# 4ment/physher

Measured on AMD Instinct MI355X. Metric: lnL+gradient evals/sec, 1000-taxon GTR+G4 fp64, 1e6 site patterns, higher is better.
Workload: dtype f64

## Files before the change

### include/physher_amd.h

```cpp
#ifndef PHYSHER_AMD_H
#define PHYSHER_AMD_H

#include <stddef.h>
#include <stdint.h>

#ifdef __cplusplus
extern "C" {
#endif

typedef struct phyamd_engine phyamd_engine;

enum {
	PHYAMD_OK = 0,
	PHYAMD_EINVAL = -1,
	PHYAMD_EDEVICE = -2,
	PHYAMD_ENOMEM = -3,
	PHYAMD_EUNSUPPORTED = -4
};

enum { PHYAMD_RESCALE_NEVER = 0, PHYAMD_RESCALE_ALWAYS = 1, PHYAMD_RESCALE_AUTO = 2 };

enum {
	PHYAMD_GRAD_FOLD_ROOT_FREQS = 1,
	PHYAMD_GRAD_COMPAT_SCALED = 2
};

typedef struct {
	int32_t tip_count;
	int32_t pattern_count;
	int32_t state_count;
	int32_t category_count;
	int32_t device;
	int32_t rescale;
	int64_t max_device_bytes;
	void *stream;
} phyamd_config;

int phyamd_create(const phyamd_config *cfg, phyamd_engine **out);
int phyamd_create_sharded(const phyamd_config *cfg, int32_t device_count, const int32_t *device_ids, phyamd_engine **out);
int phyamd_shard_count(phyamd_engine *e);
void phyamd_destroy(phyamd_engine *e);
const char *phyamd_last_error(void);
int phyamd_abi_version(void);

int phyamd_set_tip_states(phyamd_engine *e, int tip, const uint8_t *states);
int phyamd_set_tip_partials(phyamd_engine *e, int tip, const double *partials);
int phyamd_set_pattern_weights(phyamd_engine *e, const double *weights );

int phyamd_compress_patterns(int device , int32_t taxon_count, int64_t site_count, const uint8_t *const *rows,
                             const uint8_t *symbol_codes , int32_t *pattern_count, uint8_t *patterns, double *weights);

int phyamd_set_topology(phyamd_engine *e, const int32_t *left, const int32_t *right , int root);
int phyamd_set_branch_lengths(phyamd_engine *e, const double *lengths );

int phyamd_set_branch_length(phyamd_engine *e, int node, double length);
int phyamd_update_all_nodes(phyamd_engine *e);

int phyamd_store(phyamd_engine *e);
int phyamd_restore(phyamd_engine *e);

int phyamd_set_eigen(phyamd_engine *e, const double *eval, const double *evec, const double *ivec);
int phyamd_set_frequencies(phyamd_engine *e, const double *freqs );
int phyamd_set_category_rates(phyamd_engine *e, const double *rates , const double *proportions );
int phyamd_set_node_matrices(phyamd_engine *e, int node, const double *matrices);
int phyamd_set_matrices(phyamd_engine *e, const double *matrices);
int phyamd_set_rate_matrix(phyamd_engine *e, const double *Q);

int phyamd_log_likelihood(phyamd_engine *e, double *lnl);
int phyamd_gradient(phyamd_engine *e, int flags, double *lnl, double *cat_gradient);
int phyamd_branch_gradient(phyamd_engine *e, int flags, const double *rates_without_mu , double *lnl,
                           double *branch_gradient);
int phyamd_log_likelihood_device(phyamd_engine *e, double *device_out);
int phyamd_gradient_device(phyamd_engine *e, int flags, double *device_out);
int phyamd_root_invariant_term(phyamd_engine *e, double *out);

#define PHYAMD_MAX_PARAMETERS 2048
int phyamd_set_rate_matrix_derivatives(phyamd_engine *e, int count, const double *dQ);
int phyamd_parameter_gradient(phyamd_engine *e, int flags, double *lnl, double *cat_gradient, double *parameter_gradient);
int phyamd_parameter_gradient_device(phyamd_engine *e, int flags, double *device_out);
int phyamd_root_frequency_term(phyamd_engine *e, double *out );
int phyamd_branch_log_likelihood(phyamd_engine *e, int node, double length, double *lnl, double *d1, double *d2);
int phyamd_branch_hessian_diagonal(phyamd_engine *e, int flags, double *lnl, double *d1, double *d2);
int phyamd_branch_hessian_diagonal_device(phyamd_engine *e, int flags, double *device_out);
int phyamd_gradient_batch(phyamd_engine *e, int flags, int32_t count, const double *branch_lengths, double *lnl, double *cat_gradient);
int phyamd_gradient_batch_trees(phyamd_engine *e, int flags, int32_t count, const int32_t *left, const int32_t *right,
                                const int32_t *roots, const double *branch_lengths, double *lnl, double *cat_gradient);
typedef struct { int32_t items_fast, items_sequential, chunks; int64_t scratch_bytes; double ms; } phyamd_batch_profile;
int phyamd_get_batch_profile(phyamd_engine *e, phyamd_batch_profile *out);
int phyamd_nni_log_likelihoods(phyamd_engine *e, int flags, const double *central_lengths ,
                               double *lnl , double *d1 , double *d2 );
typedef struct { int32_t candidates; int64_t scratch_bytes; double ms; } phyamd_nni_profile;
int phyamd_get_nni_profile(phyamd_engine *e, phyamd_nni_profile *out);
int phyamd_spr_log_likelihoods(phyamd_engine *e, int flags, int32_t count, const int32_t *prune ,
                               double *lnl );
typedef struct { int32_t prunes, chunks; int64_t candidates, scratch_bytes; double ms; } phyamd_spr_profile;
int phyamd_get_spr_profile(phyamd_engine *e, phyamd_spr_profile *out);
int phyamd_state_posteriors(phyamd_engine *e, int flags, int32_t count, const int32_t *nodes ,
                            double *posteriors , uint8_t *states );
int phyamd_site_rate_posteriors(phyamd_engine *e, double *posteriors , double *mean_rates );
int phyamd_branch_hessian(phyamd_engine *e, int flags, double *lnl, double *gradient , double *hessian );
typedef struct { int32_t chunks; int64_t pairs, scratch_bytes; double ms; } phyamd_hessian_profile;
int phyamd_get_hessian_profile(phyamd_engine *e, phyamd_hessian_profile *out);
int phyamd_synchronize(phyamd_engine *e);

int phyamd_get_pattern_log_likelihoods(phyamd_engine *e, double *out );
int phyamd_get_partials(phyamd_engine *e, int node, int upper, double *out);
int phyamd_get_node_matrices(phyamd_engine *e, int node, int derivative, double *out );
int phyamd_post_order_parks(int32_t tip_count, const int32_t *left , const int32_t *right, int32_t root, int32_t second_slot,
                            int32_t *out , int32_t capacity);
int phyamd_is_rescaling(phyamd_engine *e);
int phyamd_set_rescaling(phyamd_engine *e, int policy);
int phyamd_set_keep_partials(phyamd_engine *e, int on);

typedef struct {
	double matrices_ms, lower_ms, upper_ms, reduce_ms;
	int32_t lower_launches, upper_launches;
	int64_t device_bytes;
	int32_t tiles;
} phyamd_profile;
int phyamd_set_reduction_levels(phyamd_engine *e, int levels);
int phyamd_set_profiling(phyamd_engine *e, int on);
int phyamd_get_profile(phyamd_engine *e, phyamd_profile *out);

#ifdef __cplusplus
}
#endif
#endif
```

### physher_amd/_lib.py

```python
from __future__ import annotations

import ctypes as C
import os

_HERE = os.path.dirname(os.path.abspath(__file__))
LIB_PATH = os.environ.get("PHYAMD_LIB") or os.path.join(_HERE, "libphysher_amd.so")

ABI_VERSION = 5

OK, EINVAL, EDEVICE, ENOMEM, EUNSUPPORTED = 0, -1, -2, -3, -4
RESCALE_NEVER, RESCALE_ALWAYS, RESCALE_AUTO = 0, 1, 2
GRAD_FOLD_ROOT_FREQS, GRAD_COMPAT_SCALED = 1, 2


class Config(C.Structure):
    _fields_ = [
        ("tip_count", C.c_int32), ("pattern_count", C.c_int32), ("state_count", C.c_int32),
        ("category_count", C.c_int32), ("device", C.c_int32), ("rescale", C.c_int32),
        ("max_device_bytes", C.c_int64), ("stream", C.c_void_p),
    ]


class Profile(C.Structure):
    _fields_ = [
        ("matrices_ms", C.c_double), ("lower_ms", C.c_double), ("upper_ms", C.c_double), ("reduce_ms", C.c_double),
        ("lower_launches", C.c_int32), ("upper_launches", C.c_int32), ("device_bytes", C.c_int64), ("tiles", C.c_int32),
    ]


class NniProfile(C.Structure):
    _fields_ = [("candidates", C.c_int32), ("scratch_bytes", C.c_int64), ("ms", C.c_double)]


class SprProfile(C.Structure):
    _fields_ = [("prunes", C.c_int32), ("chunks", C.c_int32), ("candidates", C.c_int64), ("scratch_bytes", C.c_int64), ("ms", C.c_double)]


class HessianProfile(C.Structure):
    _fields_ = [("chunks", C.c_int32), ("pairs", C.c_int64), ("scratch_bytes", C.c_int64), ("ms", C.c_double)]


class BatchProfile(C.Structure):
    _fields_ = [
        ("items_fast", C.c_int32), ("items_sequential", C.c_int32), ("chunks", C.c_int32), ("scratch_bytes", C.c_int64), ("ms", C.c_double),
    ]


_P = C.c_void_p
SYMBOLS = [
    ("phyamd_create", C.c_int, [C.POINTER(Config), C.POINTER(_P)]),
    ("phyamd_create_sharded", C.c_int, [C.POINTER(Config), C.c_int32, _P, C.POINTER(_P)]),
    ("phyamd_shard_count", C.c_int, [_P]),
    ("phyamd_destroy", None, [_P]),
    ("phyamd_last_error", C.c_char_p, []),
    ("phyamd_abi_version", C.c_int, []),
    ("phyamd_set_tip_states", C.c_int, [_P, C.c_int, _P]),
    ("phyamd_set_tip_partials", C.c_int, [_P, C.c_int, _P]),
    ("phyamd_set_pattern_weights", C.c_int, [_P, _P]),
    ("phyamd_set_topology", C.c_int, [_P, _P, _P, C.c_int]),
    ("phyamd_set_branch_lengths", C.c_int, [_P, _P]),
    ("phyamd_set_branch_length", C.c_int, [_P, C.c_int, C.c_double]),
    ("phyamd_update_all_nodes", C.c_int, [_P]),
    ("phyamd_set_eigen", C.c_int, [_P, _P, _P, _P]),
    ("phyamd_set_frequencies", C.c_int, [_P, _P]),
    ("phyamd_set_category_rates", C.c_int, [_P, _P, _P]),
    ("phyamd_set_node_matrices", C.c_int, [_P, C.c_int, _P]),
    ("phyamd_set_matrices", C.c_int, [_P, _P]),
    ("phyamd_set_rate_matrix", C.c_int, [_P, _P]),
    ("phyamd_log_likelihood", C.c_int, [_P, C.POINTER(C.c_double)]),
    ("phyamd_gradient", C.c_int, [_P, C.c_int, C.POINTER(C.c_double), _P]),
    ("phyamd_branch_gradient", C.c_int, [_P, C.c_int, _P, C.POINTER(C.c_double), _P]),
    ("phyamd_gradient_device", C.c_int, [_P, C.c_int, _P]),
    ("phyamd_log_likelihood_device", C.c_int, [_P, _P]),
    ("phyamd_root_invariant_term", C.c_int, [_P, C.POINTER(C.c_double)]),
    ("phyamd_set_rate_matrix_derivatives", C.c_int, [_P, C.c_int, _P]),
    ("phyamd_parameter_gradient", C.c_int, [_P, C.c_int, C.POINTER(C.c_double), _P, _P]),
    ("phyamd_parameter_gradient_device", C.c_int, [_P, C.c_int, _P]),
    ("phyamd_root_frequency_term", C.c_int, [_P, _P]),
    ("phyamd_branch_log_likelihood", C.c_int, [_P, C.c_int, C.c_double, C.POINTER(C.c_double), C.POINTER(C.c_double), C.POINTER(C.c_double)]),
    ("phyamd_branch_hessian_diagonal", C.c_int, [_P, C.c_int, C.POINTER(C.c_double), _P, _P]),
    ("phyamd_branch_hessian_diagonal_device", C.c_int, [_P, C.c_int, _P]),
    ("phyamd_gradient_batch", C.c_int, [_P, C.c_int, C.c_int32, _P, _P, _P]),
    ("phyamd_gradient_batch_trees", C.c_int, [_P, C.c_int, C.c_int32, _P, _P, _P, _P, _P, _P]),
    ("phyamd_get_batch_profile", C.c_int, [_P, C.POINTER(BatchProfile)]),
    ("phyamd_nni_log_likelihoods", C.c_int, [_P, C.c_int, _P, _P, _P, _P]),
    ("phyamd_get_nni_profile", C.c_int, [_P, C.POINTER(NniProfile)]),
    ("phyamd_spr_log_likelihoods", C.c_int, [_P, C.c_int, C.c_int32, _P, _P]),
    ("phyamd_get_spr_profile", C.c_int, [_P, C.POINTER(SprProfile)]),
    ("phyamd_state_posteriors", C.c_int, [_P, C.c_int, C.c_int32, _P, _P, _P]),
    ("phyamd_site_rate_posteriors", C.c_int, [_P, _P, _P]),
    ("phyamd_branch_hessian", C.c_int, [_P, C.c_int, _P, _P, _P]),
    ("phyamd_get_hessian_profile", C.c_int, [_P, C.POINTER(HessianProfile)]),
    ("phyamd_synchronize", C.c_int, [_P]),
    ("phyamd_get_pattern_log_likelihoods", C.c_int, [_P, _P]),
    ("phyamd_get_partials", C.c_int, [_P, C.c_int, C.c_int, _P]),
    ("phyamd_get_node_matrices", C.c_int, [_P, C.c_int, C.c_int, _P]),
    ("phyamd_post_order_parks", C.c_int, [C.c_int32, _P, _P, C.c_int32, C.c_int32, _P, C.c_int32]),
    ("phyamd_is_rescaling", C.c_int, [_P]),
    ("phyamd_set_rescaling", C.c_int, [_P, C.c_int]),
    ("phyamd_set_keep_partials", C.c_int, [_P, C.c_int]),
    ("phyamd_set_reduction_levels", C.c_int, [_P, C.c_int]),
    ("phyamd_set_profiling", C.c_int, [_P, C.c_int]),
    ("phyamd_get_profile", C.c_int, [_P, C.POINTER(Profile)]),
    ("phyamd_store", C.c_int, [_P]),
    ("phyamd_restore", C.c_int, [_P]),
    ("phyamd_compress_patterns", C.c_int, [C.c_int, C.c_int32, C.c_int64, _P, _P, C.POINTER(C.c_int32), _P, _P]),
]

_lib = None


def load():
    global _lib
    if _lib is not None:
        return _lib
    if not os.path.exists(LIB_PATH):
        raise ImportError(f"{LIB_PATH} is missing: build the HIP engine first (make -C physher_amd/csrc); there is no CPU fallback")
    lib = C.CDLL(LIB_PATH)
    for name, res, args in SYMBOLS:
        fn = getattr(lib, name)
        fn.restype = res
        fn.argtypes = args
    if lib.phyamd_abi_version() != ABI_VERSION:
        raise ImportError(f"ABI mismatch: library {lib.phyamd_abi_version()} != binding {ABI_VERSION}")
    _lib = lib
    return lib


class EngineError(RuntimeError):
    def __init__(self, code, message):
        super().__init__(f"physher_amd engine error {code}: {message}")
        self.code = code
```

### physher_amd/csrc/phyamd_abi.inc

```

#include <condition_variable>
#include <functional>
#include <mutex>
#include <thread>

namespace {

class ShardWorkers {
public:
	explicit ShardWorkers(int n) : done_(0), generation_(0), stop_(false) {
		for (int i = 0; i < n; i++) threads_.emplace_back([this, i] { loop(i); });
	}
	~ShardWorkers() {
		{
			std::lock_guard<std::mutex> lk(m_);
			stop_ = true;
			generation_++;
		}
		cv_.notify_all();
		for (auto &t : threads_) t.join();
	}
	void run(const std::function<void(int)> &fn) {
		std::unique_lock<std::mutex> lk(m_);
		fn_ = &fn;
// ... 542 lines not shown
int phyamd_state_posteriors(phyamd_engine *g, int flags, int32_t count, const int32_t *nodes, double *posteriors, uint8_t *states) {
	CHECK_GROUP(g);
	ensure_scratch(g, 1);
	int rc;
	if ((rc = for_shards(g, [&](Shard *s, int i) {
		     return shard_state_posteriors(s, flags, count, nodes, (size_t)g->P, posteriors ? posteriors + (size_t)g->offset[i] * g->S : nullptr,
		                                   states ? states + g->offset[i] : nullptr, g->scratch[i].data());
	     })))
		return rc;
	double lnl;
	sum_shards(g, 1, &lnl);
	post_mask_rows(lnl, (size_t)count * g->P, g->S, posteriors, states);
	return PHYAMD_OK;
}

int phyamd_site_rate_posteriors(phyamd_engine *g, double *posteriors, double *mean_rates) {
	CHECK_GROUP(g);
	if (!posteriors) return fail(PHYAMD_EINVAL, "phyamd_site_rate_posteriors: null posteriors");
	return for_shards(g, [&](Shard *s, int i) {
		return shard_site_rate_posteriors(s, posteriors + (size_t)g->offset[i] * g->C, mean_rates ? mean_rates + g->offset[i] : nullptr);
	});
}

int phyamd_branch_hessian(phyamd_engine *g, int flags, double *lnl, double *gradient, double *hessian) {
	if (!lnl || !hessian) return fail(PHYAMD_EINVAL, "phyamd_branch_hessian: null %s", !lnl ? "lnl" : "hessian");
	if (!g || g->shards.empty()) return fail(PHYAMD_EINVAL, "phyamd_branch_hessian: null engine");
	const auto t0 = std::chrono::steady_clock::now();
	int rc;
	if (group_size(g) == 1) rc = shard_branch_hessian(g->shards[0], flags, lnl, gradient, hessian);
	else {
		const size_t N = (size_t)g->N, n = 1 + N + N * N;
		ensure_scratch(g, n);
		rc = for_shards(g, [&](Shard *s, int i) {
			double *v = g->scratch[i].data();
			return shard_branch_hessian(s, flags, v, v + 1, v + 1 + N);
		});
		if (!rc) {
			std::vector<double> total(n);
			sum_shards(g, n, total.data());
			*lnl = total[0];
			if (gradient) std::memcpy(gradient, total.data() + 1, sizeof(double) * N);
			std::memcpy(hessian, total.data() + 1 + N, sizeof(double) * N * N);
			bhess_mask(*lnl, N, gradient, hessian);
		}
	}
	g->bhess_ms = std::chrono::duration<double, std::milli>(std::chrono::steady_clock::now() - t0).count();
	return rc;
}

int phyamd_get_hessian_profile(phyamd_engine *g, phyamd_hessian_profile *out) {
	CHECK_GROUP(g);
	if (!out) return fail(PHYAMD_EINVAL, "null out");
	int rc;
	if ((rc = shard_get_hessian_profile(g->shards[0], out))) return rc;
	for (int i = 1; i < group_size(g); i++) {
		phyamd_hessian_profile p;
		if ((rc = shard_get_hessian_profile(g->shards[i], &p))) return rc;
		out->chunks = std::max(out->chunks, p.chunks);
		out->scratch_bytes += p.scratch_bytes;
	}
	out->ms = g->bhess_ms;
	return PHYAMD_OK;
}

int phyamd_log_likelihood_device(phyamd_engine *g, double *device_out) {
	CHECK_GROUP(g);
	SINGLE_DEVICE_ONLY(g, "phyamd_log_likelihood_device");
	return shard_log_likelihood_device(g->shards[0], device_out);
}
int phyamd_gradient_device(phyamd_engine *g, int flags, double *device_out) {
	CHECK_GROUP(g);
	SINGLE_DEVICE_ONLY(g, "phyamd_gradient_device");
	return shard_gradient_device(g->shards[0], flags, device_out);
}
int phyamd_parameter_gradient_device(phyamd_engine *g, int flags, double *device_out) {
	CHECK_GROUP(g);
	SINGLE_DEVICE_ONLY(g, "phyamd_parameter_gradient_device");
	return shard_parameter_gradient_device(g->shards[0], flags, device_out);
}

int phyamd_branch_hessian_diagonal_device(phyamd_engine *g, int flags, double *device_out) {
	CHECK_GROUP(g);
	SINGLE_DEVICE_ONLY(g, "phyamd_branch_hessian_diagonal_device");
	return shard_branch_hessian_diagonal_device(g->shards[0], flags, device_out);
}


int phyamd_get_pattern_log_likelihoods(phyamd_engine *g, double *out) {
	CHECK_GROUP(g);
	if (!out) return fail(PHYAMD_EINVAL, "null out");
	return for_shards(g, [&](Shard *s, int i) { return shard_get_pattern_log_likelihoods(s, out + g->offset[i]); });
}

int phyamd_get_partials(phyamd_engine *g, int node, int upper, double *out) {
	CHECK_GROUP(g);
	if (group_size(g) == 1) return shard_get_partials(g->shards[0], node, upper, out);
	if (!out) return fail(PHYAMD_EINVAL, "null out");
	int rc;
	std::vector<std::vector<double>> part(group_size(g));
	if ((rc = for_shards(g, [&](Shard *s, int i) {
		     part[i].resize((size_t)g->C * s->P * g->S);
		     return shard_get_partials(s, node, upper, part[i].data());
	     })))
		return rc;
	for (int i = 0; i < group_size(g); i++) {
		const size_t ps = (size_t)(g->offset[i + 1] - g->offset[i]);
		for (int c = 0; c < g->C; c++)
			std::memcpy(out + ((size_t)c * g->P + g->offset[i]) * g->S, part[i].data() + (size_t)c * ps * g->S, sizeof(double) * ps * g->S);
	}
	return PHYAMD_OK;
}

int phyamd_get_node_matrices(phyamd_engine *g, int node, int derivative, double *out) {
	CHECK_GROUP(g);
	return shard_get_node_matrices(g->shards[0], node, derivative, out);
}

int phyamd_post_order_parks(int32_t tip_count, const int32_t *left, const int32_t *right, int32_t root, int32_t second_slot, int32_t *out, int32_t capacity) {
	if (tip_count < 2) return fail(PHYAMD_EINVAL, "tip_count must be >= 2 (got %d)", tip_count);
	if (!left || !right) return fail(PHYAMD_EINVAL, "null left or right");
	if (capacity < 0 || (capacity > 0 && !out)) return fail(PHYAMD_EINVAL, "null out with capacity %d", capacity);
	std::unique_ptr<Shard> e(new Shard());
	e->T = tip_count;
	e->N = 2 * e->T - 1;
	e->S = 4;
	e->C = 1;
	e->P = e->Ptot = 1;
	e->root = root;
	e->left.assign(left, left + e->N);
	e->right.assign(right, right + e->N);
	e->lower_park2_on = second_slot != 0;
	int rc;
	if ((rc = build_schedule(e.get()))) return rc;
	const std::vector<NodeOp> &ops = e->walk_lower_chunk_ops;
	const std::vector<int> &off = e->walk_lower_chunk_off;
	std::vector<char> is_cut_root(e->N, 0);
	for (size_t k = 1; k + 1 < off.size(); k++)
		if (off[k] > off[k - 1]) is_cut_root[ops[off[k] - 1].parent] = 1;
	int chunk = 0;
	for (int i = 0; i < (int)ops.size() && i < capacity; i++) {
		const NodeOp &o = ops[i];
		while (i >= off[chunk + 1]) chunk++;
		auto source = [&](int side) {
			if ((side ? o.kind_right : o.kind_left) != CH_CORE) return -1;
			return o.carry_in == side + 1 ? 1 : (o.lds_park & (1 << side)) ? 2 : (o.lds_park & (0x10 << side)) ? 3 : 0;
		};
		const int32_t rec[8] = {chunk, o.parent, o.left, o.right, source(0), source(1), ((o.lds_park & 4) ? 1 : 0) | ((o.lds_park & 0x40) ? 2 : 0),
		                        (is_cut_root[o.left] ? 1 : 0) | (is_cut_root[o.right] ? 2 : 0)};
		std::memcpy(out + (size_t)i * 8, rec, sizeof(rec));
	}
	return (int)ops.size();
}

int phyamd_is_rescaling(phyamd_engine *g) {
	CHECK_GROUP(g);
	int any = 0;
	for (Shard *s : g->shards) any |= shard_is_rescaling(s);
	return any;
}

int phyamd_get_profile(phyamd_engine *g, phyamd_profile *out) {
	CHECK_GROUP(g);
	if (!out) return fail(PHYAMD_EINVAL, "null out");
	int rc;
	if ((rc = shard_get_profile(g->shards[0], out))) return rc;
	for (int i = 1; i < group_size(g); i++) {
		phyamd_profile p;
		if ((rc = shard_get_profile(g->shards[i], &p))) return rc;
		out->matrices_ms = std::max(out->matrices_ms, p.matrices_ms);
		out->lower_ms = std::max(out->lower_ms, p.lower_ms);
		out->upper_ms = std::max(out->upper_ms, p.upper_ms);
		out->reduce_ms = std::max(out->reduce_ms, p.reduce_ms);
		out->device_bytes += p.device_bytes;
		out->tiles = std::max(out->tiles, p.tiles);
	}
	return PHYAMD_OK;
}

}
```

### physher_amd/csrc/phyamd_launch.inc

```

size_t gen_image_doubles(const Shard *e) {
	return e->S == 20 ? MatImage<2, 5>::SIZE : e->S == 60 ? MatImage<4, 15>::SIZE : MatImage<4, 16>::SIZE;
}

template <int RT, int KT>
void launch_matrix_images(Shard *e, int count, const double *src, double *dst, const double *rowscale) {
	hipLaunchKernelGGL((k_matrix_images<RT, KT>), dim3(count), dim3(256), 0, e->stream, e->S, src, dst, rowscale);
}

void build_matrix_images(Shard *e, int count, const double *src, double *dst, const double *rowscale = nullptr) {
	if (e->S == 20) launch_matrix_images<2, 5>(e, count, src, dst, rowscale);
	else if (e->S == 60) launch_matrix_images<4, 15>(e, count, src, dst, rowscale);
	else launch_matrix_images<4, 16>(e, count, src, dst, rowscale);
}

int update_matrices(Shard *e) {
	if (e->generic && e->state.qimg_dirty && e->have_Q && e->have_freqs) {
		build_matrix_images(e, 1, e->d_Q, e->d_imgs + (size_t)e->N * e->C * gen_image_doubles(e));
		build_matrix_images(e, 1, e->d_Q, e->d_imgs + ((size_t)e->N * e->C + 1) * gen_image_doubles(e), e->d_freqs);
		HIP_TRY(hipGetLastError());
		q_images_rebuilt(e);
	}
	if (!e->state.matrices_dirty) return PHYAMD_OK;
	if (e->have_eigen) {
// ... 173 lines not shown
		const int off = e->upper_level_off[lv], cnt = e->upper_level_off[lv + 1] - off;
		if (cnt == 0) continue;
		dim3 grid(e->nblk, cnt);
		launched++;
		hipLaunchKernelGGL((k_upper4<WAVES, SCALE, FOLD, COMPAT, PARAMS, false>), grid, block_dims(e), lds, e->stream, e->d_upper_ops + off, e->T, e->P, e->C,
		                   e->d_tipmask, e->d_lower, e->d_upper, e->d_mats, e->d_tiptab, e->d_Q, e->d_freqs, e->d_props, e->d_weights, e->d_wl, e->d_gpart,
		                   e->nblk, dpm, dptab, pc, e->N, ppart, off, op_total, (const double *)nullptr, (const int *)nullptr, (double *)nullptr);
	}
	HIP_TRY(hipGetLastError());
	e->prof.upper_launches = launched;
	return PHYAMD_OK;
}

void bisect_blocks(int lo, int hi, int levels, std::vector<int> &bounds);

size_t hess_lds(const Shard *e) {
	const size_t nw = (size_t)e->C, nacc = 2 * (size_t)((NACC + e->C - 1) / e->C);
	return sizeof(double) * ((6 + 2 * NACC) * nw * WAVE + nw * nacc * WAVE + nw * nacc);
}

int ensure_hess_storage(Shard *e) {
	if (e->d_hess && e->hess_P == e->P && e->hess_levels == e->reduce_levels) return PHYAMD_OK;
	const int nb = (e->P + WAVE - 1) / WAVE, segments = 1 << e->reduce_levels;
	std::vector<int> bounds, wg, first;
	bisect_blocks(0, nb, e->reduce_levels, bounds);
	bounds.push_back(nb);
	for (int o = 0; o < segments; o++) {
		first.push_back((int)wg.size() / 2);
		for (int b = bounds[o]; b < bounds[o + 1]; b += PPT_UPPER) {
			wg.push_back(b);
			wg.push_back(std::min(b + PPT_UPPER, bounds[o + 1]));
		}
	}
	const int nwg = (int)wg.size() / 2;
	first.push_back(nwg);
	wg.insert(wg.end(), first.begin(), first.end());
	e->d_hess_tab.release();
	e->d_hess.release();
	e->hess_P = -1;
	int rc;
	const size_t R = (size_t)2 * e->N, need = (size_t)nwg * R + 8 * R + 2 * (R + 1);
	if ((rc = e->d_hess_tab.ensure(wg.size())) || (rc = e->d_hess.ensure(need))) return rc;
	HIP_TRY(hipMemcpyAsync(e->d_hess_tab, wg.data(), sizeof(int) * wg.size(), hipMemcpyHostToDevice, e->stream));
	HIP_TRY(hipStreamSynchronize(e->stream));
	e->hess_nwg = nwg;
	e->hess_P = e->P;
	e->hess_levels = e->reduce_levels;
	return PHYAMD_OK;
}
double *hess_result(const Shard *e) { return e->d_hess + (size_t)e->hess_nwg * 2 * e->N + (size_t)8 * 2 * e->N; }
double *hess_total(const Shard *e) { return hess_result(e) + 1 + (size_t)2 * e->N; }

int finish_hess_slab(Shard *e, double *out, int launched) {
	const int R = 2 * e->N, segments = 1 << e->reduce_levels;
	double *seg = e->d_hess + (size_t)e->hess_nwg * R;
	hipLaunchKernelGGL(k_slab_segments, dim3((R + 31) / 32, 1, segments), dim3(256), 0, e->stream, e->d_hess, 1, R, (const int *)e->d_hess_tab + 2 * e->hess_nwg, seg);
	hipLaunchKernelGGL(k_slab_finish, dim3((R + 255) / 256), dim3(256), 0, e->stream, seg, segments, 1, R, (const int *)nullptr, out + 1);
	HIP_TRY(hipMemcpyAsync(out, e->d_result, sizeof(double), hipMemcpyDeviceToDevice, e->stream));
	HIP_TRY(hipGetLastError());
	e->prof.upper_launches = launched;
	return PHYAMD_OK;
}

template <int WAVES, bool SCALE>
int launch_upper_hess(Shard *e, double *out) {
	const int levels = (int)e->upper_level_off.size() - 1, R = 2 * e->N;
	const size_t lds = hess_lds(e);
	int rc;
	if ((rc = check_reference_form(e, "k_upper4"))) return rc;
	if ((rc = allow_big_lds(k_upper4<WAVES, SCALE, false, false, false, true>, lds))) return rc;
	const int op_total = (int)e->upper_ops.size();
	HIP_TRY(hipMemsetAsync(e->d_hess, 0, sizeof(double) * (size_t)e->hess_nwg * R, e->stream));
	int launched = 0;
	for (int lv = 0; lv < levels; lv++) {
		const int off = e->upper_level_off[lv], cnt = e->upper_level_off[lv + 1] - off;
		if (cnt == 0 || e->hess_nwg == 0) continue;
		launched++;
		hipLaunchKernelGGL((k_upper4<WAVES, SCALE, false, false, false, true>), dim3(e->hess_nwg, cnt), dim3(WAVE, e->C, 1), lds, e->stream, e->d_upper_ops + off, e->T,
		                   e->P, e->C, e->d_tipmask, e->d_lower, e->d_upper, e->d_mats, e->d_tiptab, e->d_Q, e->d_freqs, e->d_props, e->d_weights, e->d_wl,
		                   (double *)nullptr, 0, (const double *)nullptr, (const double *)nullptr, 0, e->N, (double *)nullptr, off, op_total, e->d_rates,
		                   (const int *)e->d_hess_tab, e->d_hess);
	}
	HIP_TRY(hipGetLastError());
	return finish_hess_slab(e, out, launched);
}

int launch_hess4(Shard *e, double *out) {
	return by_waves(e->C, [&](auto w) {
		constexpr int W = decltype(w)::value;
		return e->scaling_on ? launch_upper_hess<W, true>(e, out) : launch_upper_hess<W, false>(e, out);
	});
}

int upload_qpi(Shard *e) {
	if (!e->state.qpi_dirty) return PHYAMD_OK;
	int rc;
	if ((rc = e->d_Qpi.ensure(16))) return rc;
	double qpi[16];
	for (int i = 0; i < 4; i++)
		for (int j = 0; j < 4; j++) qpi[i * 4 + j] = e->freqs[i] * e->Q_host[i * 4 + j];
	HIP_TRY(hipMemcpyAsync(e->d_Qpi, qpi, sizeof(qpi), hipMemcpyHostToDevice, e->stream));
	HIP_TRY(hipStreamSynchronize(e->stream));
	qpi_rebuilt(e);
	return PHYAMD_OK;
}

int ensure_mask_stream(Shard *e) {
	const size_t mstride = (size_t)e->nblk_walk_upper * e->G * WAVE;
	bool grew;
	if (int rc = e->d_mstream.ensure((size_t)std::max(1, e->stream_words) * mstride, &grew)) return rc;
	if (grew) e->mstream_epoch = 0;
	if (e->mstream_epoch == e->state.tip_epoch && e->mstride == mstride && e->mstream_layout == e->stream_row_entries) return PHYAMD_OK;
	e->mstride = mstride;
	e->stream_unsupported = false;
	e->stream_ambiguous = false;
	if (e->stream_words > 0) {
		int flag = 0;
		HIP_TRY(hipMemsetAsync(e->d_stream_flag, 0, sizeof(int), e->stream));
		hipLaunchKernelGGL(k_build_mask_stream, dim3((unsigned)((mstride + 255) / 256), std::min(e->stream_words, 32768)), dim3(256), 0, e->stream, e->stream_words, e->P, mstride,
		                   (const int *)e->d_stream_row_entries, e->d_tipmask, e->d_mstream, e->d_stream_flag);
		HIP_TRY(hipGetLastError());
		HIP_TRY(hipMemcpyAsync(&flag, e->d_stream_flag, sizeof(int), hipMemcpyDeviceToHost, e->stream));
		HIP_TRY(hipStreamSynchronize(e->stream));
		e->stream_unsupported = (flag & 1) != 0;
		e->stream_ambiguous = (flag & 2) != 0;
	}
	e->mstream_epoch = e->state.tip_epoch;
	e->mstream_layout = e->stream_row_entries;
	return PHYAMD_OK;
}

int ensure_optab(Shard *e) {
	return e->d_optab.ensure((size_t)std::max<size_t>(1, e->stream_ops.size()) * e->C * OPBLK_BYTES);
}

int ensure_exponent_storage(Shard *e) {
	int rc;
	if ((rc = e->d_lexp.ensure(lower_slots(e) * e->C * e->P)) || (rc = e->d_uexp.ensure(std::max(upper_slots_held(e), upper_slots_needed(e)) * e->C * e->P)) ||
	    (rc = e->d_Ec.ensure((size_t)e->C * e->P)) || (rc = e->d_Eroot.ensure(e->P)))
		return rc;
	return PHYAMD_OK;
}
void free_exponent_storage(Shard *e) {
	e->d_lexp.release();
	e->d_uexp.release();
	e->d_Ec.release();
	e->d_Eroot.release();
}

int make_stream_buffers(Shard *e, bool lower) {
	const bool capped = e->cfg.max_device_bytes > 0;
	int rc = ensure_mask_stream(e);
	if (!rc) rc = ensure_optab(e);
	if (!rc && lower) rc = e->d_Lc.ensure((size_t)e->C * e->P);
	if (rc == PHYAMD_ENOMEM && capped) {
		(lower ? e->lower_stream_capped : e->upper_stream_capped) = true;
		return PHYAMD_OK;
	}
	if (rc || !lower || e->stream_unsupported || stream_lower_form(e) != LowerForm::CarriedExp2) return rc;
	if ((rc = ensure_exponent_storage(e)) == PHYAMD_ENOMEM && capped) {
		prefer_reference_form(e);
		free_exponent_storage(e);
		return PHYAMD_OK;
	}
	return rc;
}

int launch_lower_stream(Shard *e) {
	int rc;
	const int nb = (e->P + WAVE - 1) / WAVE, nops = (int)e->stream_ops.size();
	if (e->stream_P != e->P || e->stream_mstride != e->mstride) {
		if ((rc = upload_schedule(e))) return rc;
		if (e->stream_P != e->P || e->stream_mstride != e->mstride) return fail(PHYAMD_EDEVICE, "streamed walk: descriptors do not match the pattern storage");
	}
	hipLaunchKernelGGL(k_op_tables, dim3(nops, e->C), dim3(64), 0, e->stream, nops, e->C, (const int *)e->d_stream_op_tips, (const int *)e->d_stream_op_deep,
	                   (const int *)e->d_stream_site_tab, e->d_mats, (const double *)nullptr, reinterpret_cast<double *>(e->d_optab.get()));
	const LowerForm form = stream_lower_form(e);
	const StreamVariant v = stream_variant(form, e->scaling_on);
	const bool exp2 = v.scale == 2, scale = v.scale == 1, tf = v.tf;
	e->lower_form = form;
	const int waves = scale ? e->C : STREAM_WAVES;
	const size_t lds = (size_t)LSTREAM_LDS_PER_WAVE * waves + (scale ? sizeof(double) * 2 * e->C * WAVE : 0);
	const unsigned gx = scale ? (unsigned)nb : (unsigned)((nb + STREAM_WAVES - 1) / STREAM_WAVES) * e->C;
	const int subtrees = (int)e->walk_lower_chunk_off.size() - 2;
	const bool amb = e->stream_ambiguous;
	auto *kernel = exp2 ? (amb ? k_lower4_stream<true, 2, true> : k_lower4_stream<false, 2, true>)
	             : scale ? (amb ? k_lower4_stream<true, 1, false> : k_lower4_stream<false, 1, false>)
	             : tf    ? (amb ? k_lower4_stream<true, 0, true> : k_lower4_stream<false, 0, true>)
	                     : (amb ? k_lower4_stream<true, 0, false> : k_lower4_stream<false, 0, false>);
	for (int phase = subtrees > 0 ? 0 : 1; phase < 2; phase++)
		hipLaunchKernelGGL(kernel, dim3(gx, phase ? 1 : subtrees), dim3(WAVE, waves), lds, e->stream, (const LowerDesc *)e->d_lstream_ops,
		                   (const LowerChunk *)e->d_lstream_chunks, (const int *)e->d_walk_lower_chunk_off, phase ? std::max(0, subtrees) : 0, nops, e->P, e->C, nb,
		                   (const uint32_t *)e->d_mstream, e->mstride, e->d_lower, (const double *)e->d_mats, (const char *)e->d_optab, (const double *)e->d_freqs,
		                   (const double *)e->d_props, e->d_Lc, phase, exp2 ? reinterpret_cast<double *>(e->d_lexp.get()) : scale ? e->d_lscale : (double *)nullptr, e->xcd_map,
		                   exp2 ? e->d_Ec : (int *)nullptr);
	hipLaunchKernelGGL(k_root_finish64, dim3(nb), dim3(64), 0, e->stream, e->P, e->C, (const double *)e->d_Lc, (const double *)e->d_weights, e->d_plk, e->d_wl, e->d_lnl_part,
	                   scale ? (const double *)(e->d_lscale + (size_t)e->core_index[e->root] * e->P) : (const double *)nullptr, exp2 ? (const int *)e->d_Ec : (const int *)nullptr,
	                   exp2 ? e->d_Eroot : (int *)nullptr);
	HIP_TRY(hipGetLastError());
	e->prof.lower_launches = subtrees > 0 ? 2 : 1;
	e->lnl_blocks = nb;
	e->lnl_per_block = true;
	return PHYAMD_OK;
}

template <bool FOLD, bool SCALE>
int launch_upper_stream(Shard *e) {
	int rc;
	const int nb = (e->P + WAVE - 1) / WAVE, R = e->stream_R, nops = (int)e->stream_ops.size();
	if ((size_t)nb * e->C * R > (size_t)e->N * e->C * e->gpart_row) return fail(PHYAMD_EDEVICE, "gradient slab too small for the streamed walk");
	e->d_gslab = e->d_gpart;
	if (e->stream_P != e->P || e->stream_mstride != e->mstride) {
		if ((rc = upload_schedule(e))) return rc;
		if (e->stream_P != e->P || e->stream_mstride != e->mstride) return fail(PHYAMD_EDEVICE, "streamed walk: descriptors do not match the pattern storage");
	}
	if ((rc = e->d_oct.ensure((size_t)8 * e->C * R))) return rc;
	const StreamVariant v = stream_variant(e->lower_form, SCALE);
	if (v.scale < 0) return fail(PHYAMD_EDEVICE, "streamed walk: the stored lowers hold the %s form, which no %s post-order pass writes", form_name(e->lower_form), SCALE ? "rescaled" : "plain");
	const bool exp2 = v.scale == 2, tf = v.tf;
	if (exp2 && (rc = e->d_uexp.ensure(std::max<size_t>(1, upper_slots_held(e)) * e->C * e->P))) return rc;
	const int waves = SCALE && !exp2 ? e->C : STREAM_WAVES;
	const size_t lds = (size_t)STREAM_LDS_PER_WAVE * waves + (exp2 ? (size_t)waves * STREAM_PARK_SLOTS * WAVE * sizeof(int) : SCALE ? (size_t)4 * e->C * WAVE * sizeof(double) : 0);
	const dim3 grid_x(SCALE && !exp2 ? (unsigned)nb : (unsigned)((nb + STREAM_WAVES - 1) / STREAM_WAVES) * e->C), block(WAVE, waves);
	hipLaunchKernelGGL(k_op_tables, dim3(nops, e->C), dim3(64), 0, e->stream, nops, e->C, (const int *)e->d_stream_op_tips, (const int *)e->d_stream_op_deep,
	                   (const int *)e->d_stream_site_tab, e->d_mats, FOLD ? e->d_Q : e->d_Qpi, reinterpret_cast<double *>(e->d_optab.get()));
	const int subtrees = (int)e->walk_chunk_off.size() - 2;
	for (int phase = 0; phase < (subtrees > 0 ? 2 : 1); phase++) {
		const bool amb = e->stream_ambiguous;
		auto *kernel = exp2 ? (amb ? k_upper4_stream<FOLD, 2, true, true> : k_upper4_stream<FOLD, 2, false, true>)
		             : SCALE ? (amb ? k_upper4_stream<FOLD, 1, true, false> : k_upper4_stream<FOLD, 1, false, false>)
		             : tf    ? (amb ? k_upper4_stream<FOLD, 0, true, true> : k_upper4_stream<FOLD, 0, false, true>)
		                     : (amb ? k_upper4_stream<FOLD, 0, true, false> : k_upper4_stream<FOLD, 0, false, false>);
		hipLaunchKernelGGL(kernel, dim3(grid_x.x, phase ? subtrees : 1), block, lds, e->stream, (const StreamDesc *)e->d_stream_ops, (const StreamChunk *)e->d_stream_chunks,
		                   (const int *)e->d_walk_chunk_off, phase, nops, e->P, e->C, nb, (const uint32_t *)e->d_mstream, e->mstride, (const double *)e->d_lower, e->d_upper,
		                   (const double *)e->d_mats, (const char *)e->d_optab, (const double *)(FOLD ? e->d_Q : e->d_Qpi), (const double *)e->d_freqs, (const double *)e->d_wl,
		                   e->d_gslab, R, (const double *)e->d_props, (const double *)e->d_weights, e->xcd_map, (const int *)e->d_lexp, e->d_uexp, (const int *)e->d_Eroot);
	}
	HIP_TRY(hipGetLastError());
	e->prof.upper_launches = subtrees > 0 ? 2 : 1;
	e->grad_blocks = nb;
	e->slab_walk_order = true;
	return PHYAMD_OK;
}

void bisect_blocks(int lo, int hi, int levels, std::vector<int> &bounds) {
	if (levels == 0) {
		bounds.push_back(lo);
		return;
	}
	const int mid = lo + (hi - lo) / 2;
	bisect_blocks(lo, mid, levels - 1, bounds);
	bisect_blocks(mid, hi, levels - 1, bounds);
}

int reduce_block_sums(Shard *e, int which, const double *slab, int nb, int C, int R, const int *row_of, double *out) {
	int rc;
	const int segments = 1 << e->reduce_levels;
	if ((rc = e->d_oct_lo.ensure(20)) || (rc = e->d_oct.ensure((size_t)8 * C * R))) return rc;
	int *table = e->d_oct_lo + 10 * which;
	if (e->seg_nb[which] != nb || e->seg_levels[which] != e->reduce_levels) {
		std::vector<int> bounds;
		bisect_blocks(0, std::min(nb, (e->P + WAVE - 1) / WAVE), e->reduce_levels, bounds);
		bounds.push_back(nb);
		HIP_TRY(hipMemcpyAsync(table, bounds.data(), sizeof(int) * bounds.size(), hipMemcpyHostToDevice, e->stream));
		HIP_TRY(hipStreamSynchronize(e->stream));
		e->seg_nb[which] = nb;
		e->seg_levels[which] = e->reduce_levels;
	}
	hipLaunchKernelGGL(k_slab_segments, dim3((R + 31) / 32, C, segments), dim3(256), 0, e->stream, slab, C, R, (const int *)table, e->d_oct);
	hipLaunchKernelGGL(k_slab_finish, dim3((C * R + 255) / 256), dim3(256), 0, e->stream, e->d_oct, segments, C, R, row_of, out);
	HIP_TRY(hipGetLastError());
	return PHYAMD_OK;
}

int reduce_stream_slab(Shard *e, double *out) {
	HIP_TRY(hipMemsetAsync(out, 0, sizeof(double) * (size_t)e->N * e->C, e->stream));
	return reduce_block_sums(e, 1, e->d_gslab, e->grad_blocks, e->C, e->stream_R, (const int *)e->d_stream_qnode, out);
}

template <int WAVES, bool FOLD, bool SCALE, bool COMPAT>
int launch_upper_walk_v(Shard *e) {
	const int ops = (int)e->walk_upper_ops.size(), nb = e->nblk_walk_upper * e->G;
	int rc;
	if ((rc = check_reference_form(e, "k_upper4_walk"))) return rc;
	const size_t lds = sizeof(double) * ((size_t)e->G * e->C * NACC * WCOL + (SCALE ? (size_t)4 * e->G * e->C * WAVE : 0) + (size_t)4 * e->G * e->C * WAVE);
	if ((rc = allow_big_lds(k_upper4_walk<WAVES, FOLD, false, SCALE, COMPAT>, lds))) return rc;
	const int subtrees = (int)e->walk_chunk_off.size() - 2;
	for (int phase = 0; phase < (subtrees > 0 ? 2 : 1); phase++)
		hipLaunchKernelGGL((k_upper4_walk<WAVES, FOLD, false, SCALE, COMPAT>), dim3(e->nblk_walk_upper, phase ? subtrees : 1), block_dims(e), lds, e->stream,
		                   e->d_walk_chunk_ops, ops, e->T, e->P, e->C, e->d_tipmask, e->d_lower, e->d_upper, e->d_mats, e->d_tiptab, FOLD ? e->d_Q : e->d_Qpi,
		                   e->d_freqs, e->d_wl, e->d_gpart, nb, (const double *)nullptr, (const double *)nullptr, (double *)nullptr, e->d_props, e->d_weights,
		                   (const int *)e->d_walk_chunk_off, phase);
	HIP_TRY(hipGetLastError());
	e->prof.upper_launches = subtrees > 0 ? 2 : 1;
	e->grad_blocks = nb;
	return PHYAMD_OK;
}

template <int WAVES>
int launch_upper_walk(Shard *e, bool fold, bool compat) {
	if (e->scaling_on) {
		if (fold) return compat ? launch_upper_walk_v<WAVES, true, true, true>(e) : launch_upper_walk_v<WAVES, true, true, false>(e);
		return compat ? launch_upper_walk_v<WAVES, false, true, true>(e) : launch_upper_walk_v<WAVES, false, true, false>(e);
	}
	return fold ? launch_upper_walk_v<WAVES, true, false, false>(e) : launch_upper_walk_v<WAVES, false, false, false>(e);
}

std::vector<double> eigen_basis_derivatives(const Shard *e) {
	const int S = e->S;
	const double *evec = e->model.data() + S, *ivec = e->model.data() + S + S * S;
	std::vector<double> B((size_t)e->np * S * S), tmp((size_t)S * S);
	for (int th = 0; th < e->np; th++) {
		const double *dQ = e->dQ_host.data() + (size_t)th * S * S;
		for (int a = 0; a < S; a++)
			for (int j = 0; j < S; j++) {
				double v = 0.0;
				for (int i = 0; i < S; i++) v += ivec[a * S + i] * dQ[i * S + j];
				tmp[a * S + j] = v;
			}
		for (int a = 0; a < S; a++)
			for (int b = 0; b < S; b++) {
				double v = 0.0;
				for (int j = 0; j < S; j++) v += tmp[a * S + j] * evec[j * S + b];
				B[((size_t)th * S + a) * S + b] = v;
			}
	}
	return B;
}

template <int WAVES, bool SCALE>
int launch_upper_walk_params(Shard *e) {
	const int ops = (int)e->walk_upper_ops.size(), nb = e->nblk_walk_upper * e->G, S = 4, np = e->np;
	const size_t lds = sizeof(double) * ((size_t)e->G * e->C * 16 * WCOL + (SCALE ? (size_t)4 * e->G * e->C * WAVE : 0));
	int rc;
	if ((rc = check_reference_form(e, "k_upper4_walk (parameters)"))) return rc;
	if ((rc = e->d_Bw.ensure((size_t)np * 16)) || (rc = e->d_pbuf.ensure(96)) || (rc = e->d_Fw.ensure((size_t)e->N * e->C * 20)) ||
	    (rc = e->d_gacc.ensure((size_t)16 * nb * e->C + 16)))
		return rc;
	{
		const double *evec = e->model.data() + S, *ivec = e->model.data() + S + S * S;
		const std::vector<double> B = eigen_basis_derivatives(e);
		std::vector<double> pb(96);
		for (int a = 0; a < 4; a++)
			for (int i = 0; i < 4; i++) {
				pb[a * 4 + i] = evec[i * 4 + a] * e->freqs[i];
				pb[16 + a * 4 + i] = ivec[a * 4 + i];
			}
		for (int m = 0; m < 16; m++)
			for (int b = 0; b < 4; b++) {
				double v = 0.0;
				for (int j = 0; j < 4; j++)
					if (m >> j & 1) v += ivec[b * 4 + j];
				pb[32 + m * 4 + b] = v;
			}
		HIP_TRY(hipMemcpyAsync(e->d_Bw, B.data(), sizeof(double) * B.size(), hipMemcpyHostToDevice, e->stream));
		HIP_TRY(hipMemcpyAsync(e->d_pbuf, pb.data(), sizeof(double) * pb.size(), hipMemcpyHostToDevice, e->stream));
		HIP_TRY(hipStreamSynchronize(e->stream));
	}
	const int nf = e->N * e->C * 20;
	hipLaunchKernelGGL(k_eigen_weights, dim3((nf + 255) / 256), dim3(256), 0, e->stream, e->C, e->N, e->d_model, e->d_rates, e->d_props, e->d_lengths, e->d_explicit,
	                   e->root, e->d_Fw);
	if constexpr (!SCALE && WAVES == 4) {
		const size_t lds4 = sizeof(double) * (size_t)4 * 16 * WCOL;
		hipLaunchKernelGGL((k_upper4_walk<4, false, true, false, false, true>), dim3((unsigned)((nb + 3) / 4) * e->C), dim3(WAVE, 1, 4), lds4, e->stream,
		                   e->d_walk_upper_ops, ops, e->T, e->P, e->C, e->d_tipmask, e->d_lower, e->d_upper, e->d_mats, e->d_tiptab, e->d_Qpi, e->d_freqs, e->d_wl,
		                   e->d_gpart, nb, e->d_pbuf, e->d_Fw, e->d_gacc, e->d_props, e->d_weights, (const int *)nullptr, 0);
	} else
		hipLaunchKernelGGL((k_upper4_walk<WAVES, false, true, SCALE, false>), dim3(e->nblk_walk_upper), block_dims(e), lds, e->stream, e->d_walk_upper_ops, ops, e->T,
		                   e->P, e->C, e->d_tipmask, e->d_lower, e->d_upper, e->d_mats, e->d_tiptab, e->d_Qpi, e->d_freqs, e->d_wl, e->d_gpart, nb, e->d_pbuf, e->d_Fw,
		                   e->d_gacc, e->d_props, e->d_weights, (const int *)nullptr, 0);
	double *gsum = e->d_gacc + (size_t)16 * nb * e->C;
	hipLaunchKernelGGL(k_reduce_rows, dim3(16), dim3(64), 0, e->stream, e->d_gacc, nb * e->C, (const uint8_t *)nullptr, gsum);
	hipLaunchKernelGGL(k_contract_parameters, dim3((np + 63) / 64), dim3(64), 0, e->stream, np, e->d_Bw, gsum, e->d_result + 1 + (size_t)e->N * e->C);
	HIP_TRY(hipGetLastError());
	e->prof.upper_launches = 1;
	e->grad_blocks = nb;
	return PHYAMD_OK;
}

template <int WAVES>
int launch_upper_w(Shard *e, int flags, PassKernel k) {
	const bool fold = flags & PHYAMD_GRAD_FOLD_ROOT_FREQS, compat = (flags & PHYAMD_GRAD_COMPAT_SCALED) && e->scaling_on;
	e->grad_blocks = e->nblk;
	if (k == PassKernel::Walk) return launch_upper_walk<WAVES>(e, fold, compat);
	if (e->scaling_on) {
		if (fold) return compat ? launch_upper_levels<WAVES, true, true, true, false>(e) : launch_upper_levels<WAVES, true, true, false, false>(e);
		return compat ? launch_upper_levels<WAVES, true, false, true, false>(e) : launch_upper_levels<WAVES, true, false, false, false>(e);
	}
	return fold ? launch_upper_levels<WAVES, false, true, false, false>(e) : launch_upper_levels<WAVES, false, false, false, false>(e);
// ... 233 lines not shown
```

### physher_amd/csrc/phyamd_schedule.inc

```

int bind_device(Shard *e) {
	HIP_TRY(hipSetDevice(e->device));
	return PHYAMD_OK;
}

size_t node_partial_doubles(const Shard *e) { return (size_t)e->C * e->S * (e->generic ? e->Pp : e->P); }
size_t lower_slots(const Shard *e) { return e->d_lower.size() / node_partial_doubles(e); }
size_t upper_slots_held(const Shard *e) { return e->d_upper.size() / node_partial_doubles(e); }

constexpr int WALK_CHUNKS = 3;
void build_walk_chunks(Shard *e) {
	const std::vector<NodeOp> &src = e->walk_upper_ops;
	const int n = (int)src.size(), N = e->N;
	e->walk_chunk_ops = src;
	e->walk_chunk_off.assign({0, n});
	e->walk_chunk_slots = 0;
	if (n == 0) return;
	std::vector<int> opi(N, -1), size(n, 1);
	for (int i = 0; i < n; i++) opi[src[i].parent] = i;
	for (int i = n - 1; i >= 0; i--)
		for (int ch : {src[i].left, src[i].right})
			if (opi[ch] >= 0) size[i] += size[opi[ch]];
	const int target = std::max(16, (n + WALK_CHUNKS - 1) / WALK_CHUNKS);
	std::vector<char> top(n, 0), cut(n, 0);
// ... 45 lines not shown
			else {
				kind[w] = INTERNAL;
				std::vector<int> &fl = free_list[k];
				if (!fl.empty()) {
					local[w] = fl.back();
					fl.pop_back();
				} else
					local[w] = next_local[k]++;
			}
		}
		if (freed >= 0) free_list[k].push_back(freed);
	}
	std::vector<int> base(chunks + 1, 0);
	for (int k = 0; k < chunks; k++) base[k + 1] = base[k] + next_local[k];
	const int slots = base[chunks] + cross;
	for (int i = 0; i < n; i++)
		for (int side = 0; side < 2; side++) {
			const int ch = side ? src[i].right : src[i].left, j = opi[ch];
			if (j < 0) continue;
			const int w = i * 2 + side, lds_bit = side ? 4 : 2;
			int32_t &slot = side ? ops[i].upper_slot_right : ops[i].upper_slot_left;
			if (kind[w] == NONE) slot = -1;
			else if (kind[w] == LDS) {
				slot = -1;
				ops[j].upper_slot_parent = -1;
			} else {
				slot = kind[w] == INTERNAL ? base[chunk_of[i]] + local[w] : base[chunks] + local[w];
				ops[i].lds_park &= ~lds_bit;
				if (kind[w] == CROSS) {
					ops[i].lds_park &= ~(side ? 0x40 : 0x20);
					ops[j].lds_park &= ~0x10;
				}
				ops[j].carry_in = 0;
				ops[j].upper_slot_parent = slot;
				ops[j].lds_park &= ~1;
			}
		}
	e->walk_chunk_ops.clear();
	e->walk_chunk_off.assign(1, 0);
	for (int i = 0; i < n; i++)
		if (top[i] && !cut[i]) e->walk_chunk_ops.push_back(ops[i]);
	e->walk_chunk_off.push_back((int)e->walk_chunk_ops.size());
	std::vector<int> cuts;
	for (int j = 0; j < n; j++)
		if (cut[j]) cuts.push_back(j);
	std::stable_sort(cuts.begin(), cuts.end(), [&](int a, int b) { return size[a] > size[b]; });
	for (int j : cuts) {
		for (int i = j; i < j + size[j]; i++) e->walk_chunk_ops.push_back(ops[i]);
		e->walk_chunk_off.push_back((int)e->walk_chunk_ops.size());
	}
	e->walk_chunk_slots = slots;
	e->walk_upper_slots = std::max(e->walk_upper_slots, slots);
}

void build_lower_walk_chunks(Shard *e) {
	const std::vector<NodeOp> &src = e->walk_lower_ops;
	const int n = (int)src.size(), N = e->N;
	e->walk_lower_chunk_ops = src;
	e->walk_lower_chunk_off.assign({0, n});
	if (n == 0) return;
	std::vector<int> opi(N, -1), size(n, 1);
	for (int i = 0; i < n; i++) opi[src[i].parent] = i;
	for (int i = 0; i < n; i++)
		for (int ch : {src[i].left, src[i].right})
			if (opi[ch] >= 0) size[i] += size[opi[ch]];
	const int target = std::max(16, (n + WALK_CHUNKS - 1) / WALK_CHUNKS);
	if (n < 32) return;
	std::vector<char> cut(n, 0), in_cut(n, 0);
	std::vector<int> stack{n - 1};
	while (!stack.empty()) {
		const int i = stack.back();
		stack.pop_back();
		for (int ch : {src[i].left, src[i].right}) {
			const int j = opi[ch];
			if (j < 0) continue;
			if (size[j] > target) stack.push_back(j);
			else cut[j] = 1;
		}
	}
	std::vector<NodeOp> out;
	std::vector<int> off{0}, cuts, at(n, -1);
	for (int j = 0; j < n; j++)
		if (cut[j]) cuts.push_back(j);
	std::stable_sort(cuts.begin(), cuts.end(), [&](int a, int b) { return size[a] > size[b]; });
	for (int j : cuts) {
		for (int i = j - size[j] + 1; i <= j; i++) {
			in_cut[i] = 1;
			at[i] = (int)out.size();
			out.push_back(src[i]);
		}
		out[off.back()].carry_in = 0;
		off.push_back((int)out.size());
	}
	int prev = -1;
	for (int i = 0; i < n; i++) {
		if (in_cut[i]) continue;
		NodeOp op = src[i];
		const int jl = opi[op.left], jr = opi[op.right];
		const bool next_to_cut = (jl >= 0 && cut[jl]) || (jr >= 0 && cut[jr]);
		op.carry_in = prev >= 0 && prev == op.left ? 1 : prev >= 0 && prev == op.right ? 2 : 0;
		if (next_to_cut) {
			for (int side = 0; side < 2; side++) {
				const int j = side ? jr : jl;
				if (op.lds_park & (side ? 2 : 1)) out[at[j]].lds_park &= ~4;
				if (op.lds_park & (side ? 0x20 : 0x10)) out[at[j]].lds_park &= ~0x40;
			}
			op.lds_park &= ~0x33;
		}
		at[i] = (int)out.size();
		out.push_back(op);
		prev = op.parent;
	}
	off.push_back((int)out.size());
	e->walk_lower_chunk_ops = out;
	e->walk_lower_chunk_off = off;
}

struct MaskPacker {
	std::vector<int> &rows;
	int row = -1, used = 32, entries = 8;
	explicit MaskPacker(std::vector<int> &r) : rows(r), row((int)r.size() / 8 - 1) {}
	void add(const int *tips, int &out_row, int &out_shift) {
		int span = 0, n = 0;
		for (int j = 0; j < 6; j++)
			if (tips[j] >= 0) {
				span = j + 1;
				n++;
			}
		const int bits = 1 + 4 * span;
		if (used + bits > 32 || entries + n > 8) {
			rows.insert(rows.end(), 8, -1);
			row++;
			used = 0;
			entries = 0;
		}
		out_row = row;
		out_shift = used;
		for (int j = 0; j < 6; j++)
			if (tips[j] >= 0) rows[(size_t)row * 8 + entries++] = tips[j] | (used + 1 + 4 * j) << 20 | used << 25;
		used += bits;
	}
};

void build_stream_ops(Shard *e) {
	const int n = (int)e->walk_chunk_ops.size();
	e->stream_ops.assign(n, StreamOp{});
	e->stream_chunks.clear();
	e->stream_row_entries.clear();
	e->stream_site_tab.assign((size_t)n * 16, -1);
	e->stream_op_tips.assign((size_t)n * 12, -1);
	e->stream_op_deep.assign(n, 0);
	e->stream_qnode.clear();
	e->stream_words = 0;
	if (n == 0) return;
	std::vector<NodeOp> src = e->walk_chunk_ops;
	std::vector<char> chunk_start(n + 1, 0);
	for (int off : e->walk_chunk_off) chunk_start[off] = 1;
	std::vector<char> from_prev(n, 0);
	for (int i = 1; i < n; i++) {
		const NodeOp &o = src[i];
		NodeOp &pv = src[i - 1];
		const bool proot = o.upper_slot_parent < 0 && !o.carry_in && !(o.lds_park & 1);
		if (chunk_start[i] || proot || o.carry_in || (o.lds_park & 0x11) || o.upper_slot_parent < 0) continue;
		if (pv.upper_slot_left == o.upper_slot_parent) {
			pv.carry_out = 1;
			pv.upper_slot_left = -1;
			from_prev[i] = 1;
		} else if (pv.upper_slot_right == o.upper_slot_parent) {
			pv.carry_out = 2;
			pv.upper_slot_right = -1;
			from_prev[i] = 1;
		}
	}
	for (NodeOp &o : src)
		if (o.carry_out == 2) {
			std::swap(o.left, o.right);
			std::swap(o.core_left, o.core_right);
			std::swap(o.kind_left, o.kind_right);
			std::swap(o.lt0, o.rt0);
			std::swap(o.lt1, o.rt1);
			std::swap(o.lt2, o.rt2);
			std::swap(o.linner, o.rinner);
			std::swap(o.upper_slot_left, o.upper_slot_right);
			o.lds_park = (o.lds_park & 0x11) | ((o.lds_park & 2) ? 4 : 0) | ((o.lds_park & 4) ? 2 : 0) | ((o.lds_park & 0x20) ? 0x40 : 0) | ((o.lds_park & 0x40) ? 0x20 : 0);
			o.carry_out = 1;
		}
	auto half_kind = [](int k) { return k == CH_TIP ? HK_TIP : k == CH_CHERRY ? HK_CHERRY : HK_CHERRY_TIP; };
	std::vector<int> first_word(n, -1), words(n, 0), same_row(n, 0), want_a(n, -1), want_b(n, -1), want_u(n, -1);
	MaskPacker packer(e->stream_row_entries);
	for (int i = 0; i < n; i++) {
		const NodeOp &o = src[i];
		StreamOp &s = e->stream_ops[i];
		const bool proot = o.upper_slot_parent < 0 && !o.carry_in && !(o.lds_park & 1) && !from_prev[i];
		int fl = (o.kind_left & 7) | (o.kind_right & 7) << 3;
		fl |= ((o.lds_park & 2) ? 1 : (o.lds_park & 4) ? 2 : 0) << 12;
		s.parent = o.parent;
		s.slot_parent = o.upper_slot_parent;
		s.slot_left = o.upper_slot_left;
		s.slot_right = o.upper_slot_right;
		const bool lds2_on = STREAM_PARK_SLOTS > 1;
		if (lds2_on && (o.lds_park & 0x60)) {
			fl |= ((o.lds_park & 0x20) ? 1 : 2) << 12 | 1 << 6;
			((o.lds_park & 0x20) ? s.slot_left : s.slot_right) = -1;
		}
		s.lnode = o.left;
		s.rnode = o.right;
		for (int side = 0; side < 2; side++) {
			const int kind = side ? o.kind_right : o.kind_left, node = side ? o.right : o.left;
			int32_t *a = side ? s.ra : s.la;
			for (int j = 0; j < 10; j++) a[j] = -1;
			int tips[8] = {-1, -1, -1, -1, -1, -1, -1, -1};
			if (kind == CH_TIP) tips[0] = node;
			else if (kind == CH_CHERRY || kind == CH_CHERRY_TIP) {
				a[0] = side ? o.rt0 : o.lt0;
				a[1] = side ? o.rt1 : o.lt1;
				a[2] = side ? o.rt2 : o.lt2;
				a[3] = side ? o.rinner : o.linner;
				tips[0] = a[0];
				tips[1] = a[1];
				if (kind == CH_CHERRY_TIP) tips[2] = a[2];
			} else if (kind == CH_DEEP) {
				const DeepDesc &d = e->deep_host[node];
				e->stream_op_deep[i] |= 1 << side;
				for (int h = 0; h < 2; h++) {
					const int hk = h ? d.kind_right : d.kind_left;
					int32_t *q = a + 5 * h;
					q[0] = h ? d.right : d.left;
					q[1] = h ? d.rt0 : d.lt0;
					q[2] = h ? d.rt1 : d.lt1;
					q[3] = h ? d.rt2 : d.lt2;
					q[4] = h ? d.rinner : d.linner;
					fl |= half_kind(hk) << (16 + 4 * side + 2 * h);
					if (hk == CH_TIP) tips[3 * h] = q[0];
					else {
						tips[3 * h] = q[1];
						tips[3 * h + 1] = q[2];
						if (hk == CH_CHERRY_TIP) tips[3 * h + 2] = q[3];
					}
				}
			}
			for (int j = 0; j < 6; j++) e->stream_op_tips[(size_t)i * 12 + 6 * side + j] = tips[j];
			if (kind != CH_CORE) {
				int row, shift;
				packer.add(tips, row, shift);
				if (words[i] == 0) first_word[i] = row;
				else same_row[i] = row == first_word[i];
				s.wsh |= shift << (5 * words[i]);
				words[i]++;
			}
		}
		int usrc;
		if (o.kind_left == CH_CORE) want_a[i] = o.core_left;
		if (o.kind_right == CH_CORE) want_b[i] = o.core_right;
		if (proot) usrc = SU_ROOT;
		else if (o.carry_in || from_prev[i]) usrc = SU_CARRY;
		else if (o.lds_park & 1) usrc = SU_LDS;
		else if (lds2_on && (o.lds_park & 0x10)) {
			usrc = SU_LDS;
			fl |= 1 << 7;
		} else {
			usrc = SU_U;
			want_u[i] = o.upper_slot_parent;
		}
		fl |= usrc << 9;
		s.flags = fl;
		const int sites[10] = {o.left, o.kind_left >= CH_CHERRY ? o.lt0 : -1, o.kind_left >= CH_CHERRY ? o.lt1 : -1, o.kind_left == CH_CHERRY_TIP ? o.linner : -1,
		                       o.right, o.kind_right >= CH_CHERRY ? o.rt0 : -1, o.kind_right >= CH_CHERRY ? o.rt1 : -1, o.kind_right == CH_CHERRY_TIP ? o.rinner : -1,
		                       o.kind_left == CH_CHERRY_TIP ? o.lt2 : -1, o.kind_right == CH_CHERRY_TIP ? o.rt2 : -1};
		for (int j = 0; j < 10; j++)
			if (sites[j] >= 0) {
				e->stream_site_tab[(size_t)i * 16 + j] = 8 * (int)e->stream_qnode.size();
				e->stream_qnode.push_back(sites[j]);
			}
	}
	e->stream_R = (int)e->stream_qnode.size();
	e->stream_words = (int)e->stream_row_entries.size() / 8;
	const int chunks = (int)e->walk_chunk_off.size() - 1;
	for (int k = 0; k < chunks; k++) {
		const int b = e->walk_chunk_off[k], en = e->walk_chunk_off[k + 1];
		StreamChunk ch{-1, 0, -1, -1, -1, 0, {0, 0}};
		if (b < en) ch = StreamChunk{first_word[b], words[b], want_a[b], want_b[b], want_u[b], same_row[b], {0, 0}};
		e->stream_chunks.push_back(ch);
		for (int i = b; i < en; i++) {
			StreamOp &s = e->stream_ops[i];
			const bool last = i + 1 == en;
			s.nx_mask_word = last ? -1 : first_word[i + 1];
			s.flags |= (last ? 0 : words[i + 1]) << 14;
			s.flags |= (!last && src[i + 1].kind_right != CH_CORE ? 1 : 0) << 24;
			s.flags |= (!last && same_row[i + 1] ? 1 : 0) << 25;
			s.nx_a = last ? -1 : want_a[i + 1];
			s.nx_b = last ? -1 : want_b[i + 1];
			s.nx_u = last ? -1 : want_u[i + 1];
		}
	}
	e->stream_P = e->P;
	e->stream_mstride = (size_t)e->nblk_walk_upper * e->G * WAVE;
	const int64_t plane_bytes = (int64_t)e->P * 4 * 8, array_bytes = plane_bytes * e->C, row_bytes = (int64_t)e->stream_mstride * 4;
	e->stream_desc.assign(n, StreamDesc{});
	for (int i = 0; i < n; i++) {
		const StreamOp &s = e->stream_ops[i];
		StreamDesc &d = e->stream_desc[i];
		auto moff = [&](int32_t node) { return node >= 0 ? node * e->C * 128 : 0; };
		const int kinds[2] = {s.flags & 7, (s.flags >> 3) & 7};
		d.flags = s.flags;
		d.parent = moff(s.parent);
		d.lnode = moff(s.lnode);
		d.rnode = moff(s.rnode);
		for (int side = 0; side < 2; side++) {
			const int32_t *a = side ? s.ra : s.la;
			int32_t *m = side ? d.rm : d.lm;
			for (int j = 0; j < 5; j++) m[j] = 0;
			if (kinds[side] == CH_DEEP) {
				m[0] = moff(a[0]);
				m[1] = moff(a[4]);
				m[2] = moff(a[5]);
				m[3] = moff(a[9]);
			} else if (kinds[side] == CH_CHERRY_TIP)
				m[4] = moff(a[3]);
		}
		d.nx_words = s.nx_mask_word >= 0 ? (int64_t)s.nx_mask_word * row_bytes : 0;
		d.nx_a = s.nx_a >= 0 ? (int64_t)s.nx_a * array_bytes : 0;
		d.nx_b = s.nx_b >= 0 ? (int64_t)s.nx_b * array_bytes : 0;
		d.nx_u = s.nx_u >= 0 ? (int64_t)s.nx_u * array_bytes : 0;
		d.st_left = s.slot_left >= 0 ? (int64_t)s.slot_left * array_bytes : 0;
		d.st_right = s.slot_right >= 0 ? (int64_t)s.slot_right * array_bytes : 0;
		d.wsh = s.wsh;
		d.flags |= (s.nx_a >= 0 ? 1 << 26 : 0) | (s.nx_b >= 0 ? 1 << 27 : 0) | (s.nx_u >= 0 ? 1 << 28 : 0) | (s.slot_left >= 0 ? 1 << 29 : 0) | (s.slot_right >= 0 ? 1 << 30 : 0);
	}
}

void build_lower_stream_ops(Shard *e) {
	const int n = (int)e->walk_lower_chunk_ops.size(), ns = (int)e->stream_ops.size();
	e->lstream_desc.clear();
	e->lstream_chunks.clear();
	if (n == 0 || ns == 0) return;
	std::vector<int> sop(e->N, -1);
	for (int i = 0; i < ns; i++) sop[e->walk_chunk_ops[i].parent] = i;
	for (const NodeOp &o : e->walk_lower_chunk_ops)
		if (sop[o.parent] < 0) return;
	const int64_t plane_bytes = (int64_t)e->P * 4 * 8, array_bytes = plane_bytes * e->C, row_bytes = (int64_t)e->stream_mstride * 4;
	auto moff = [&](int32_t node) { return node >= 0 ? node * e->C * 128 : 0; };
	e->lstream_desc.assign(n, LowerDesc{});
	std::vector<int> pieces(n, 0), first_word(n, 0), last_word(n, 0), words(n, 0);
	MaskPacker packer(e->stream_row_entries);
	for (int i = 0; i < n; i++) {
		const NodeOp &o = e->walk_lower_chunk_ops[i];
		const StreamOp &u = e->stream_ops[sop[o.parent]];
		LowerDesc &d = e->lstream_desc[i];
		const int kinds[2] = {u.flags & 7, (u.flags >> 3) & 7};
		for (int side = 0; side < 2; side++)
			if (kinds[side] != CH_CORE) {
				int row, shift;
				packer.add(&e->stream_op_tips[(size_t)sop[o.parent] * 12 + 6 * side], row, shift);
				if (words[i] == 0) first_word[i] = row;
				last_word[i] = row;
				d.wsh |= shift << (5 * words[i]) | (row & 3) << (10 + 2 * words[i]);
				words[i]++;
			}
		int fl = (u.flags & 0x3F) | (u.flags & 0x00FF0000);
		d.lnode = moff(u.lnode);
		d.rnode = moff(u.rnode);
		d.self = o.parent == e->root ? 0 : moff(o.parent);
		d.store = (int64_t)o.core_parent * array_bytes;
		d.ls_store = (int64_t)o.core_parent * e->P * 8;
		for (int side = 0; side < 2; side++) {
			const int32_t *a = side ? u.ra : u.la;
			int32_t *m = side ? d.rm : d.lm;
			for (int j = 0; j < 5; j++) m[j] = 0;
			if (kinds[side] == CH_DEEP) {
				m[0] = moff(a[0]);
				m[1] = moff(a[4]);
				m[2] = moff(a[5]);
				m[3] = moff(a[9]);
			} else if (kinds[side] == CH_CHERRY_TIP)
				m[4] = moff(a[3]);
			if (kinds[side] != CH_CORE) continue;
			const int ch = side ? u.rnode : u.lnode;
			const bool is_left = ch == o.left;
			int src = 0;
			if (o.carry_in == (is_left ? 1 : 2)) src = 1;
			else if (o.lds_park & (is_left ? 1 : 2)) src = 2;
			else if (o.lds_park & (is_left ? 0x10 : 0x20)) src = 3;
			if (src == 0 || src == 3) {
				(side ? d.mem_r : d.mem_l) = (int64_t)e->core_index[ch] * array_bytes;
				(side ? d.ls_r : d.ls_l) = (int64_t)e->core_index[ch] * e->P * 8;
			}
			fl |= src << (6 + 2 * side);
		}
		if (o.lds_park & 4) fl |= 1 << 10;
		if (o.lds_park & 0x40) fl |= 1 << 26;
		pieces[i] = (kinds[0] != CH_CORE ? 1 : 0) | (kinds[1] != CH_CORE ? 2 : 0);
		d.flags = fl;
	}
	const int chunks = (int)e->walk_lower_chunk_off.size() - 1;
	for (int k = 0; k < chunks; k++) {
		const int b = e->walk_lower_chunk_off[k], en = e->walk_lower_chunk_off[k + 1];
		LowerChunk ch{0, 0, 0, 0, 0};
		int have = -1;
		auto fresh_rows = [&](int i, int &first) {
			if (words[i] == 0) return 0;
			first = have < 0 ? first_word[i] : std::max(first_word[i], have + 1);
			const int count = last_word[i] - first + 1;
			have = std::max(have, last_word[i]);
			return std::max(0, count);
		};
		if (b < en) {
			const int si = sop[e->walk_lower_chunk_ops[b].parent];
			int first = 0;
			const int count = fresh_rows(b, first);
			ch = LowerChunk{si, pieces[b], count, first & 3, (int64_t)first * row_bytes};
		}
		e->lstream_chunks.push_back(ch);
		for (int i = b; i < en; i++) {
			LowerDesc &d = e->lstream_desc[i];
			const bool last = i + 1 == en;
			const int sn = last ? 0 : sop[e->walk_lower_chunk_ops[i + 1].parent];
			d.nx_block = sn;
			int first = 0;
			const int count = last ? 0 : fresh_rows(i + 1, first);
			d.nx_words = (int64_t)first * row_bytes;
			d.flags |= count << 14;
			d.flags |= (first & 3) << 12;
			d.flags |= (last ? 0 : ((pieces[i + 1] & 2) ? 1 : 0)) << 24;
			d.flags |= (last ? 0 : (pieces[i + 1] & 1)) << 25;
		}
	}
	e->stream_words = (int)e->stream_row_entries.size() / 8;
}

int build_schedule(Shard *e) {
	const int N = e->N, T = e->T;
	e->parent.assign(N, -1);
	std::vector<int> seen(N, 0);
	for (int n = 0; n < N; n++) {
		const int l = e->left[n], r = e->right[n];
		if (n < T) {
			if (l != -1 || r != -1) return fail(PHYAMD_EINVAL, "node %d is a tip (id < tip_count) but has children", n);
			continue;
		}
		if (l < 0 || r < 0 || l >= N || r >= N || l == r) return fail(PHYAMD_EINVAL, "internal node %d has invalid children (%d, %d)", n, l, r);
		if (++seen[l] > 1 || ++seen[r] > 1) return fail(PHYAMD_EINVAL, "node %d or %d has two parents", l, r);
		e->parent[l] = n;
// ... 153 lines not shown
		}
		std::vector<int> lower_op_of(N, -1);
		std::vector<Frame> st{{e->root, 0}};
		while (!st.empty()) {
			Frame &f = st.back();
			const int n = f.node, l = e->left[n], r = e->right[n];
			const int first = csize[l] >= csize[r] ? l : r, second = first == l ? r : l;
			if (f.stage == 0) {
				f.stage = 1;
				if (kind[first] == CH_CORE) st.push_back({first, 0});
			} else if (f.stage == 1) {
				f.stage = 2;
				if (kind[second] == CH_CORE) st.push_back({second, 0});
			} else {
				NodeOp op = make_op(n);
				op.carry_in = 0;
				if (!e->walk_lower_ops.empty()) {
					const int prev = e->walk_lower_ops.back().parent;
					if (prev == l) op.carry_in = 1;
					else if (prev == r) op.carry_in = 2;
				}
				op.lds_park = 0;
				if (kind[first] == CH_CORE && kind[second] == CH_CORE && lower_op_of[first] >= 0) {
					if (!two_core[second]) {
						e->walk_lower_ops[lower_op_of[first]].lds_park |= 4;
						op.lds_park |= first == l ? 1 : 2;
					} else if (e->lower_park2_on && lparks[second] == 1) {
						e->walk_lower_ops[lower_op_of[first]].lds_park |= 0x40;
						op.lds_park |= first == l ? 0x10 : 0x20;
					}
				}
				lower_op_of[n] = (int)e->walk_lower_ops.size();
				e->walk_lower_ops.push_back(op);
				st.pop_back();
			}
		}
		std::vector<uint8_t> parks(N, 0), in_lds(N, 0), in_lds2(N, 0);
		std::vector<int> height(N, 0);
		for (int i = N - 1; i >= 0; i--) {
			const int n = order[i];
			if (kind[n] != CH_CORE && kind[n] != CH_DEEP) continue;
			const int l = e->left[n], r = e->right[n];
			const bool lo = kind[l] == CH_CORE || kind[l] == CH_DEEP, ro = kind[r] == CH_CORE || kind[r] == CH_DEEP;
			parks[n] = (lo && ro) || (lo && parks[l]) || (ro && parks[r]);
			if (lo && ro) {
				const int first = usize[l] <= usize[r] ? l : r, second = first == l ? r : l;
				height[n] = std::max(1 + height[first], height[second]);
			} else
				height[n] = lo ? height[l] : ro ? height[r] : 0;
		}
		std::vector<int> free_w;
		int next_w = 0;
		std::vector<int> slot_of(N, -1);
		std::vector<int> stack2{e->root};
		int carried_node = -1;
		while (!stack2.empty()) {
			const int n = stack2.back();
			stack2.pop_back();
			NodeOp op = make_op(n);
			op.carry_in = (n != e->root && carried_node == n) ? 1 : 0;
			op.upper_slot_parent = -1;
			op.lds_park = 0;
			if (n != e->root && !op.carry_in) {
				op.upper_slot_parent = slot_of[n];
				free_w.push_back(slot_of[n]);
				if (in_lds[n]) op.lds_park |= 1;
				if (in_lds2[n]) op.lds_park |= 0x10;
			}
			const int l = e->left[n], r = e->right[n];
			const bool lc = kind[l] == CH_CORE || kind[l] == CH_DEEP, rc2 = kind[r] == CH_CORE || kind[r] == CH_DEEP;
			int first = -1, second = -1;
			if (lc && rc2) {
				first = usize[l] <= usize[r] ? l : r;
				second = first == l ? r : l;
			} else if (lc || rc2)
				first = lc ? l : r;
			op.carry_out = first < 0 ? 0 : (first == l ? 1 : 2);
			carried_node = first;
			if (second >= 0) {
				int sl;
				if (free_w.size() > 1 || (free_w.size() == 1 && free_w.back() != op.upper_slot_parent)) {
					size_t pick = free_w.size() - 1;
					if (free_w[pick] == op.upper_slot_parent) pick--;
					sl = free_w[pick];
					free_w.erase(free_w.begin() + pick);
				} else
					sl = next_w++;
				slot_of[second] = sl;
				(second == l ? op.upper_slot_left : op.upper_slot_right) = sl;
				if (!parks[first]) {
					in_lds[second] = 1;
					op.lds_park |= second == l ? 2 : 4;
				} else if (height[first] == 1) {
					in_lds2[second] = 1;
					op.lds_park |= second == l ? 0x20 : 0x40;
				}
				stack2.push_back(second);
			}
			if (first >= 0) stack2.push_back(first);
			e->walk_upper_ops.push_back(op);
		}
		e->walk_upper_slots = next_w;
		if (e->walking) {
			build_walk_chunks(e);
			build_lower_walk_chunks(e);
		}
	}
	return PHYAMD_OK;
}

int ensure_lower_storage(Shard *e) {
	const size_t need = (size_t)std::max(1, e->core_count) * (e->two_slots ? 2 : 1);
	if (lower_slots(e) >= need) return PHYAMD_OK;
	e->d_lower.release();
	e->d_lscale.release();
	return e->d_lower.ensure(need * node_partial_doubles(e));
}

void refresh_op_cores(Shard *e) {
	for (std::vector<NodeOp> *ops : {&e->lower_ops, &e->upper_ops, &e->walk_lower_ops, &e->walk_upper_ops, &e->walk_chunk_ops, &e->walk_lower_chunk_ops})
		for (NodeOp &op : *ops) {
			op.core_parent = e->core_index[op.parent];
			op.core_left = e->core_index[op.left];
			op.core_right = e->core_index[op.right];
		}
}

int upload_schedule(Shard *e) {
	int rc;
	if ((rc = e->d_lower_ops.ensure(e->N)) || (rc = e->d_upper_ops.ensure(e->N))) return rc;
	HIP_TRY(hipMemcpyAsync(e->d_lower_ops, e->lower_ops.data(), e->lower_ops.size() * sizeof(NodeOp), hipMemcpyHostToDevice, e->stream));
	HIP_TRY(hipMemcpyAsync(e->d_upper_ops, e->upper_ops.data(), e->upper_ops.size() * sizeof(NodeOp), hipMemcpyHostToDevice, e->stream));
	static_assert(sizeof(DeepDesc) == 6 * sizeof(double), "DeepDesc is laid out in the tail of the tip-message table");
	if (!e->generic)
		HIP_TRY(hipMemcpyAsync(e->d_tiptab + (size_t)e->T * e->C * 64, e->deep_host.data(), e->deep_host.size() * sizeof(DeepDesc), hipMemcpyHostToDevice,
		                       e->stream));
	if (e->walking || e->gen_walking) {
		if ((rc = e->d_walk_lower_ops.ensure(e->N)) || (rc = e->d_walk_upper_ops.ensure(e->N))) return rc;
		HIP_TRY(hipMemcpyAsync(e->d_walk_lower_ops, e->walk_lower_ops.data(), e->walk_lower_ops.size() * sizeof(NodeOp), hipMemcpyHostToDevice, e->stream));
		HIP_TRY(hipMemcpyAsync(e->d_walk_upper_ops, e->walk_upper_ops.data(), e->walk_upper_ops.size() * sizeof(NodeOp), hipMemcpyHostToDevice, e->stream));
	}
	if (e->walking) {
		if ((rc = e->d_walk_chunk_ops.ensure(e->N)) || (rc = e->d_walk_chunk_off.ensure((size_t)e->N + 2))) return rc;
		HIP_TRY(hipMemcpyAsync(e->d_walk_chunk_ops, e->walk_chunk_ops.data(), e->walk_chunk_ops.size() * sizeof(NodeOp), hipMemcpyHostToDevice, e->stream));
		HIP_TRY(hipMemcpyAsync(e->d_walk_chunk_off, e->walk_chunk_off.data(), e->walk_chunk_off.size() * sizeof(int), hipMemcpyHostToDevice, e->stream));
		if ((rc = e->d_walk_lower_chunk_ops.ensure(e->N)) || (rc = e->d_walk_lower_chunk_off.ensure((size_t)e->N + 2))) return rc;
		HIP_TRY(hipMemcpyAsync(e->d_walk_lower_chunk_ops, e->walk_lower_chunk_ops.data(), e->walk_lower_chunk_ops.size() * sizeof(NodeOp), hipMemcpyHostToDevice, e->stream));
		HIP_TRY(hipMemcpyAsync(e->d_walk_lower_chunk_off, e->walk_lower_chunk_off.data(), e->walk_lower_chunk_off.size() * sizeof(int), hipMemcpyHostToDevice, e->stream));
		if (stream_possible(e)) {
			build_stream_ops(e);
			build_lower_stream_ops(e);
			if ((rc = e->d_stream_ops.ensure(e->N)) || (rc = e->d_stream_chunks.ensure((size_t)e->N + 2)) || (rc = e->d_stream_row_entries.ensure((size_t)e->N * 32)) ||
			    (rc = e->d_stream_site_tab.ensure((size_t)e->N * 16)) || (rc = e->d_stream_qnode.ensure(e->N)) || (rc = e->d_stream_op_tips.ensure((size_t)e->N * 12)) ||
			    (rc = e->d_stream_flag.ensure(1)) || (rc = e->d_stream_op_deep.ensure(e->N)))
				return rc;
			HIP_TRY(hipMemcpyAsync(e->d_stream_op_tips, e->stream_op_tips.data(), e->stream_op_tips.size() * sizeof(int), hipMemcpyHostToDevice, e->stream));
			HIP_TRY(hipMemcpyAsync(e->d_stream_op_deep, e->stream_op_deep.data(), e->stream_op_deep.size() * sizeof(int), hipMemcpyHostToDevice, e->stream));
			HIP_TRY(hipMemcpyAsync(e->d_stream_ops, e->stream_desc.data(), e->stream_desc.size() * sizeof(StreamDesc), hipMemcpyHostToDevice, e->stream));
			HIP_TRY(hipMemcpyAsync(e->d_stream_chunks, e->stream_chunks.data(), e->stream_chunks.size() * sizeof(StreamChunk), hipMemcpyHostToDevice, e->stream));
			HIP_TRY(hipMemcpyAsync(e->d_stream_row_entries, e->stream_row_entries.data(), e->stream_row_entries.size() * sizeof(int), hipMemcpyHostToDevice, e->stream));
			HIP_TRY(hipMemcpyAsync(e->d_stream_site_tab, e->stream_site_tab.data(), e->stream_site_tab.size() * sizeof(int), hipMemcpyHostToDevice, e->stream));
			HIP_TRY(hipMemcpyAsync(e->d_stream_qnode, e->stream_qnode.data(), e->stream_qnode.size() * sizeof(int), hipMemcpyHostToDevice, e->stream));
			if ((rc = e->d_lstream_ops.ensure(e->N)) || (rc = e->d_lstream_chunks.ensure((size_t)e->N + 2))) return rc;
			HIP_TRY(hipMemcpyAsync(e->d_lstream_ops, e->lstream_desc.data(), e->lstream_desc.size() * sizeof(LowerDesc), hipMemcpyHostToDevice, e->stream));
			HIP_TRY(hipMemcpyAsync(e->d_lstream_chunks, e->lstream_chunks.data(), e->lstream_chunks.size() * sizeof(LowerChunk), hipMemcpyHostToDevice, e->stream));
		}
	}
	std::vector<uint8_t> valid((size_t)e->N * e->C, 1);
	for (int c = 0; c < e->C; c++) valid[(size_t)e->root * e->C + c] = 0;
	HIP_TRY(hipMemcpyAsync(e->d_row_valid, valid.data(), valid.size(), hipMemcpyHostToDevice, e->stream));
	HIP_TRY(hipStreamSynchronize(e->stream));
	return PHYAMD_OK;
}

size_t upper_slots_needed(const Shard *e) {
	const bool level_path = !e->walking || e->level_upper_needed;
	return (size_t)std::max(1, level_path ? std::max(e->upper_slots, e->walk_upper_slots) : e->walk_upper_slots);
}

int ensure_upper_storage(Shard *e, PassKernel k) {
	if (k == PassKernel::Levels) e->level_upper_needed = true;
	return e->d_upper.ensure(upper_slots_needed(e) * node_partial_doubles(e));
}

int ensure_scaling_storage(Shard *e) { return e->d_lscale.ensure(lower_slots(e) * e->P); }

int check_ready(Shard *e) {
	if (!e->have_topology) return fail(PHYAMD_EINVAL, "phyamd_set_topology has not been called");
	if (!e->have_lengths) return fail(PHYAMD_EINVAL, "phyamd_set_branch_lengths has not been called");
	if (!e->have_freqs) return fail(PHYAMD_EINVAL, "phyamd_set_frequencies has not been called");
	if (!e->have_rates) return fail(PHYAMD_EINVAL, "phyamd_set_category_rates has not been called");
	if (!e->have_weights) return fail(PHYAMD_EINVAL, "phyamd_set_pattern_weights has not been called");
	for (int t = 0; t < e->T; t++)
		if (!e->tip_set[t]) return fail(PHYAMD_EINVAL, "tip %d has no data (phyamd_set_tip_states / phyamd_set_tip_partials)", t);
	if (!e->have_eigen) {
		for (int n = 0; n < e->N; n++)
			if (n != e->root && !e->explicit_host[n]) return fail(PHYAMD_EINVAL, "no eigen system and node %d has no explicit matrices", n);
	}
	return PHYAMD_OK;
}
```

### physher_amd/csrc/phyamd_shard.inc

```

enum class LowerForm { Reference, Carried, CarriedExp2 };

struct ScheduleCounts { int core_count, upper_slots, widest; };

struct Shard {
	phyamd_config cfg{};
	DeviceBudget mem;
	DeviceBudget tile_mem{&mem};
	int T = 0, N = 0, P = 0, S = 0, C = 0, root = -1;
	int G = 1;
	bool generic = false;
	int Pp = 0;
	int nblk_root = 0;
	int nblk_lower = 0;
	int nblk_walk = 0, nblk_walk_upper = 0;
	int lower_walk_slots[2] = {0, 0};
	int gen_slots[3][2] = {};
	int lnl_blocks = 0;
	int grad_blocks = 0;
	size_t gpart_row = 0;
	struct State {
		bool all_dirty = true;
		std::vector<int> changed;
		bool force_root = false;
		bool upper_valid = false;
		int path_node = -1;
		bool matrices_dirty = true;
		bool qimg_dirty = true;
		bool qpi_dirty = true;
		int qp_kind = -1;
		bool params_dirty = true;
		bool stored_valid = false;
		bool tiled_eval_done = false;
		bool tiled_root_term = false;
		unsigned long tip_epoch = 1;
		bool spr_lists_dirty = true;
	} state;
	bool incremental_pass = false;
	std::vector<NodeOp> inc_ops;
	std::vector<int> inc_level_off;
	DeviceArray<NodeOp> d_inc_ops{&mem};
	const std::vector<int> *act_level_off = nullptr;
	NodeOp *act_lower_ops = nullptr;
	bool level_upper_needed = false;
	struct Stored {
		std::vector<double> lengths, model, freqs, rates, props;
		std::vector<int32_t> core_index;
		bool have_eigen = false, scaling_on = false;
		unsigned long epoch = 0;
		double lnl = 0.0;
	} stored;
	int Ptot = 0, tiles = 1;
	DeviceArray<uint8_t> d_tip_all{&tile_mem};
	DeviceArray<double> d_weights_all{&tile_mem}, d_plk_all{&tile_mem}, d_total{&tile_mem};
	unsigned long schedule_epoch = 0;
	bool two_slots = false;
	bool generic_fusion = true;
	bool walk_enabled = true;
	bool walking = false, gen_walking = false;
	DeviceArray<int> d_gen_walk_counter{&mem};
	int gen_walk_slots[1] = {0};
	std::vector<NodeOp> walk_lower_ops, walk_upper_ops;
	DeviceArray<NodeOp> d_walk_lower_ops{&mem}, d_walk_upper_ops{&mem};
	int walk_upper_slots = 0;
	std::vector<NodeOp> walk_chunk_ops;
	std::vector<int> walk_chunk_off;
	int walk_chunk_slots = 0;
	std::vector<NodeOp> walk_lower_chunk_ops;
	std::vector<int> walk_lower_chunk_off;
	DeviceArray<NodeOp> d_walk_lower_chunk_ops{&mem};
	DeviceArray<int> d_walk_lower_chunk_off{&mem};
	DeviceArray<NodeOp> d_walk_chunk_ops{&mem};
	DeviceArray<int> d_walk_chunk_off{&mem};
	bool upper_stream_capped = false;
	bool lower_stream_capped = false;
	int xcd_map = 1;
	std::vector<StreamOp> stream_ops;
	std::vector<StreamDesc> stream_desc;
	int stream_P = 0;
	size_t stream_mstride = 0;
	std::vector<StreamChunk> stream_chunks;
	std::vector<LowerDesc> lstream_desc;
	std::vector<LowerChunk> lstream_chunks;
	DeviceArray<LowerDesc> d_lstream_ops{&mem};
	DeviceArray<LowerChunk> d_lstream_chunks{&mem};
	std::vector<int> stream_row_entries;
	std::vector<int> stream_site_tab;
	std::vector<int> stream_qnode;
	std::vector<int> stream_op_tips;
	std::vector<int> stream_op_deep;
	DeviceArray<int> d_stream_op_tips{&mem}, d_stream_flag{&mem}, d_stream_op_deep{&mem};
	DeviceArray<char> d_optab{&mem};
	bool stream_ambiguous = false;
	bool stream_unsupported = false;
	int stream_words = 0, stream_R = 0;
	DeviceArray<StreamDesc> d_stream_ops{&mem};
	DeviceArray<StreamChunk> d_stream_chunks{&mem};
	DeviceArray<int> d_stream_row_entries{&mem}, d_stream_site_tab{&mem}, d_stream_qnode{&mem}, d_oct_lo{&mem};
	DeviceArray<uint32_t> d_mstream{&tile_mem};
	size_t mstride = 0;
	unsigned long mstream_epoch = 0;
	std::vector<int> mstream_layout;
	double *d_gslab = nullptr;
	DeviceArray<double> d_oct{&mem};
	bool slab_walk_order = false;
	int reduce_levels = 3, seg_nb[2] = {-1, -1}, seg_levels[2] = {-1, -1};
	bool lnl_per_block = false;
	DeviceArray<double> d_Lc{&tile_mem};
	DeviceArray<double> d_imgs{&mem};
	DeviceArray<double> d_qp_mats{&mem};
	DeviceArray<double> d_qp_imgs{&mem};
	DeviceArray<double> d_inv_part{&tile_mem};
	int device = 0;
	hipStream_t stream = nullptr;
	bool own_stream = false;

	std::vector<int32_t> left, right, parent;
	std::vector<double> lengths, model, freqs, rates, props;
	std::vector<uint8_t> explicit_host;
	bool have_topology = false, have_lengths = false, have_eigen = false, have_freqs = false, have_rates = false, have_weights = false;
	std::vector<uint8_t> tip_set;
	bool scaling_on = false;
	LowerForm lower_form = LowerForm::Reference;
	bool reference_form_only = false;
	bool exp2_on = true, tform_on = true;
	bool lower_park2_on = true;
	DeviceArray<int> d_lexp{&tile_mem}, d_uexp{&tile_mem}, d_Ec{&tile_mem}, d_Eroot{&tile_mem};
	bool keep_partials = false;
	bool profiling = false;
	bool prof_pending = false, prof_with_upper = false;

	std::vector<NodeOp> lower_ops, upper_ops;
	std::vector<int> lower_level_off, upper_level_off;
	std::vector<int32_t> upper_slot;
	int upper_slots = 0;
	std::vector<int32_t> core_index;
	int core_count = 0;
	ScheduleCounts scaled_counts{0, 0, 1};
	bool have_scaled_counts = false;
	bool fusion_enabled = true, fused = false;
	std::vector<DeepDesc> deep_host;
	int deep_count = 0;

	DeviceArray<uint8_t> d_tipmask{&tile_mem};
	DeviceArray<unsigned long long> d_tipsets{&mem};
	std::vector<unsigned long long> tipsets_host;
	size_t tipsets_uploaded = 0;
	DeviceArray<double> d_lower{&tile_mem}, d_upper{&tile_mem}, d_mats{&mem}, d_dmats{&mem};
	DeviceArray<double> d_Q{&mem};
	DeviceArray<double> d_Qpi{&mem};
	std::vector<double> Q_host;
	bool have_Q = false;
	DeviceArray<double> d_tiptab{&mem};
	int np = 0;
	std::vector<double> dQ_host;
	DeviceArray<double> d_B{&mem};
	DeviceArray<double> d_dpm{&mem};
	DeviceArray<double> d_dptab{&mem};
	DeviceArray<double> d_ppart{&mem};
	DeviceArray<double> d_Bw{&mem};
	DeviceArray<double> d_pbuf{&mem};
	DeviceArray<double> d_Fw{&mem};
	DeviceArray<double> d_gacc{&mem};
	std::vector<int> node_kind;
	DeviceArray<PathStep> d_path_steps{&mem};
	DeviceArray<double> d_path_upper{&mem}, d_path_tmp{&mem}, d_path_lower{&mem};
	DeviceArray<double> d_path_side{&mem};
	DeviceArray<double> d_pg_lower{&mem};
	DeviceArray<int> d_hess_tab{&tile_mem};
	DeviceArray<double> d_hess{&tile_mem};
	int hess_nwg = 0, hess_P = -1, hess_levels = -1;
	DeviceArray<double> d_hess_invf{&mem};
	int gen_hess_slots[2] = {0, 0};
	DeviceArray<double> d_branch{&mem};
	bool upper_fold = false;
	DeviceArray<double> d_rf_part{&mem};
	DeviceArray<double> d_gen_scratch{&mem};
	DeviceArray<int> d_pg_nodes{&mem}, d_pg_core{&mem};
	DeviceArray<double> d_pg_den{&mem}, d_pg_Gw{&mem}, d_pg_B{&mem};
	DeviceArray<double> d_model{&mem}, d_freqs{&mem}, d_rates{&mem}, d_props{&mem}, d_lengths{&mem}, d_result{&mem};
	DeviceArray<double> d_weights{&tile_mem}, d_plk{&tile_mem}, d_lscale{&tile_mem}, d_lnl_part{&tile_mem}, d_gpart{&tile_mem};
	DeviceArray<double> d_wl{&tile_mem};
	DeviceArray<uint8_t> d_explicit{&mem}, d_row_valid{&mem};
	DeviceArray<NodeOp> d_lower_ops{&mem}, d_upper_ops{&mem};
	double *h_result = nullptr;
	double *h_lengths = nullptr;
	hipEvent_t ev_lengths = nullptr;
	hipEvent_t ev_check = nullptr;
	bool check_pending = false;
	int nblk = 0;

	hipEvent_t ev[5] = {nullptr, nullptr, nullptr, nullptr, nullptr};
	phyamd_profile prof{};

	std::vector<uint8_t> tip_empty;
	int batch_max_patterns = 0;
	bool batch_trace = false;
	std::vector<int32_t> batch_left, batch_right;
	int batch_root = -1, batch_upper_slots = 0;
	std::vector<BatchOp> batch_ops;
	DeviceArray<BatchOp> d_batch_ops{&mem};
	DeviceBudget batch_mem{&mem};
	DeviceArray<double> d_batch_len{&batch_mem}, d_batch_mats{&batch_mem}, d_batch_out{&batch_mem};
	DeviceArray<double> d_batch_lower{&batch_mem}, d_batch_upper{&batch_mem}, d_batch_slab{&batch_mem}, d_batch_lnl{&batch_mem};
	DeviceArray<BatchOp> d_batch_item_ops{&batch_mem};
	DeviceArray<int32_t> d_batch_roots{&batch_mem};
	int batch_items = 0;
	bool batch_grad = false;
	int batch_slots = 0;
	bool batch_trees = false;
	bool batch_nni = false;
	phyamd_batch_profile batch_prof{};
	DeviceArray<BatchOp> d_nni_ops{&batch_mem};
	DeviceArray<NniCand> d_nni_cands{&batch_mem};
	DeviceArray<int32_t> d_nni_cand_of{&batch_mem};
	DeviceArray<double> d_nni_len{&batch_mem}, d_nni_mats{&batch_mem};
	DeviceArray<double> d_nni_slab{&batch_mem}, d_nni_out{&batch_mem};
	bool nni_lists_valid = false;
	phyamd_nni_profile nni_prof{};
	std::vector<BatchOp> spr_ops;
	std::vector<int32_t> spr_tin, spr_tout, spr_lower_at, spr_upper_at;
	DeviceArray<SprCand> d_spr_cands{&batch_mem};
	DeviceArray<int32_t> d_spr_cand_of{&batch_mem};
	DeviceArray<double> d_spr_slab{&batch_mem}, d_spr_out{&batch_mem};
	DeviceArray<double> d_spr_len{&batch_mem}, d_spr_mats{&batch_mem};
	bool batch_spr = false;
	phyamd_spr_profile spr_prof{};
	DeviceArray<PostRow> d_post_rows{&mem};
	DeviceArray<double> d_post_out{&mem}, d_post_lower{&mem};
	DeviceArray<uint8_t> d_post_states{&mem};
	DeviceArray<double> d_bhess_tan{&batch_mem}, d_bhess_rows{&batch_mem}, d_bhess_tiles{&batch_mem}, d_bhess_sums{&batch_mem};
	DeviceArray<char> d_bhess_lists{&batch_mem};
	phyamd_hessian_profile bhess_prof{};
};

enum class Input { TipData, PatternWeights, Topology, BranchLengths, BranchLength, Eigen, RateMatrix, Frequencies, CategoryRates, NodeMatrices,
                   Matrices, RateMatrixDerivatives, UpdateAllNodes, ScheduleRebuilt };

bool lowers_current(const Shard *e) { return !e->state.all_dirty && e->state.changed.empty() && !e->state.force_root; }
bool uppers_resident(const Shard *e) { return e->keep_partials && e->state.upper_valid; }
bool tiled_totals_current(const Shard *e, bool root_term = false) { return e->state.tiled_eval_done && (!root_term || e->state.tiled_root_term); }

void uppers_dropped(Shard *e) { e->state.upper_valid = false, e->state.path_node = -1; }
void lowers_discarded(Shard *e) { e->state.all_dirty = true, uppers_dropped(e); }

// ... 125 lines not shown
```

### physher_amd/csrc/phyamd_shard_api.inc

```

ScheduleCounts schedule_counts(const Shard *e) {
	ScheduleCounts c{e->core_count, std::max(e->upper_slots, e->walk_upper_slots), 1};
	for (size_t i = 0; i + 1 < e->lower_level_off.size(); i++) c.widest = std::max(c.widest, e->lower_level_off[i + 1] - e->lower_level_off[i]);
	for (size_t i = 0; i + 1 < e->upper_level_off.size(); i++) c.widest = std::max(c.widest, e->upper_level_off[i + 1] - e->upper_level_off[i]);
	return c;
}

double tile_working_set(const Shard *e, double p, bool exact, const ScheduleCounts &k) {
	const double pp = e->S == 4 ? p : std::ceil(p / 16.0) * 16.0, npd = (double)e->C * e->S * pp;
	const double per_pattern = (double)e->T * p + 8.0 * p * (3.0 + (e->S == 4 ? 0.0 : (double)e->C));
	const bool may_scale = e->cfg.rescale != PHYAMD_RESCALE_NEVER, exponents = may_scale && e->S == 4 && e->exp2_on;
	if (!exact) return 8.0 * (exponents ? 1.125 : 1.0) * ((e->S == 4 ? 0.5 : 1.6) * (double)(e->N - e->T) * npd + 2.0 * npd) + per_pattern;
	double doubles = (double)(std::max(1, k.core_count) + std::max(1, k.upper_slots)) * npd;
	if (may_scale) doubles += (double)std::max(1, k.core_count) * p + (e->S == 4 ? 0.0 : 5.0 * k.widest * e->C * p);
	if (exponents) doubles += 0.5 * ((double)(std::max(1, k.core_count) + std::max(1, k.upper_slots) + 1) * e->C * p + p);
	if (e->S == 4) doubles += (double)e->C * p;
	doubles += (double)e->N * e->C * (p / (WAVE * std::max(1, 4 / e->C)) + 1.0);
	if (e->S == 4) doubles += 2.0 * e->N * (p / (WAVE * PPT_UPPER) + 19.0) + 0.5 * p / 64.0;
	return 8.0 * doubles + per_pattern;
}

double tile_working_set(const Shard *e, double p, bool exact) {
	const double now = tile_working_set(e, p, exact, schedule_counts(e));
	return e->have_scaled_counts ? std::max(now, tile_working_set(e, p, exact, e->scaled_counts)) : now;
}

double walk_reserve(const Shard *e) {
	if (e->S != 4) return 0.0;
	return std::max(0.0, (double)e->N * e->C * OPBLK_BYTES - (double)e->d_optab.size()) + std::max(0.0, 8.0 * (8.0 * e->C * e->N - (double)e->d_oct.size()));
}

int choose_tiles(Shard *e, bool exact) {
	double cap = (double)e->cfg.max_device_bytes;
	const bool automatic = e->cfg.max_device_bytes <= 0;
	const double tile_sized = (double)(e->tile_mem.bytes - (int64_t)(e->d_hess.bytes() + e->d_hess_tab.bytes() + e->d_mstream.bytes() +
	                                                                   (e->C < 2 ? e->d_inv_part.bytes() : 0)));
	if (automatic) {
		size_t free_bytes = 0, total_bytes = 0;
		cap = hipMemGetInfo(&free_bytes, &total_bytes) == hipSuccess ? 0.92 * ((double)free_bytes + tile_sized) : 0.0;
	} else
		cap -= (double)e->mem.bytes - tile_sized + 65536.0 + walk_reserve(e);
	if (!automatic && cap <= 0)
		return fail(PHYAMD_ENOMEM, "max_device_bytes (%lld) does not even hold what is resident whatever the tile size (%lld bytes)",
		            (long long)e->cfg.max_device_bytes, (long long)(e->mem.bytes - (int64_t)tile_sized));
	e->P = e->Ptot;
	e->tiles = 1;
	if (cap > 0 && tile_working_set(e, (double)e->Ptot, exact) > cap) {
		const double resident = (double)e->T * e->Ptot + 16.0 * e->Ptot;
		int tiles = 2, per = 0;
		for (;; tiles++) {
			per = ((e->Ptot + tiles - 1) / tiles + 255) / 256 * 256;
			if (tile_working_set(e, (double)per, exact) + resident <= cap) break;
			if (per <= 256)
				return fail(PHYAMD_ENOMEM, "%s (%.3g bytes) is below the smallest tiled working set (%.3g bytes)",
				            automatic ? "free device memory" : "max_device_bytes", cap, tile_working_set(e, 256.0, exact) + resident);
		}
		e->P = per;
		e->tiles = (e->Ptot + per - 1) / per;
	}
	return PHYAMD_OK;
}

int allocate_pattern_storage(Shard *e) {
	e->G = std::max(1, 4 / e->C);
	e->nblk = (e->P + WAVE * e->G * PPT_UPPER - 1) / (WAVE * e->G * PPT_UPPER);
	e->nblk_lower = (e->P + WAVE * e->G * PPT_LOWER - 1) / (WAVE * e->G * PPT_LOWER);
	{
		const int groups = (e->P + WAVE * e->G - 1) / (WAVE * e->G);
		e->lower_walk_slots[0] = e->lower_walk_slots[1] = 0;
		e->nblk_walk = groups;
		e->nblk_walk_upper = groups;
	}
	if (e->generic) {
		e->Pp = (e->P + 15) / 16 * 16;
		const int ppb = e->S == 20 ? GenGeo<2>::MIN_PATTERNS_PER_BLOCK : GenGeo<4>::MIN_PATTERNS_PER_BLOCK;
		e->nblk = (e->P + ppb - 1) / ppb;
		e->nblk_lower = e->nblk;
		e->nblk_root = (e->P + 255) / 256;
	}
	int rc;
	if ((rc = e->d_tipmask.ensure((size_t)e->T * e->P + 8))) return rc;
	if (e->tiles > 1) {
		if ((rc = e->d_tip_all.ensure((size_t)e->T * e->Ptot)) || (rc = e->d_weights_all.ensure(e->Ptot)) || (rc = e->d_plk_all.ensure(e->Ptot)) ||
		    (rc = e->d_total.ensure((size_t)1 + e->N * e->C + 2 * PHYAMD_MAX_PARAMETERS)))
			return rc;
	}
	if ((rc = e->d_weights.ensure(e->P)) || (rc = e->d_plk.ensure(e->P)) || (rc = e->d_wl.ensure(e->P))) return rc;
	if ((rc = e->d_lnl_part.ensure(std::max(std::max(std::max(e->nblk, e->nblk_lower), (e->nblk_walk_upper + 2) * e->G), e->nblk_root))))
		return rc;
	if (e->generic && (rc = e->d_Lc.ensure((size_t)e->C * e->P))) return rc;
	if (e->C >= 2 && (rc = e->d_inv_part.ensure((size_t)(e->P + 255) / 256 + 1))) return rc;
	e->gpart_row = (size_t)std::max(e->nblk, e->generic ? 0 : e->nblk_walk_upper * e->G);
	if ((rc = e->d_gpart.ensure((size_t)e->N * e->C * e->gpart_row))) return rc;
	HIP_TRY(hipMemsetAsync(e->d_gpart, 0, sizeof(double) * (size_t)e->N * e->C * e->gpart_row, e->stream));
	HIP_TRY(hipStreamSynchronize(e->stream));
	return PHYAMD_OK;
}

void free_pattern_storage(Shard *e) {
	e->tile_mem.release_all();
	e->batch_mem.release_all();
	e->d_gslab = nullptr;
	e->hess_P = -1;
	e->mstream_epoch = 0;
}

void shard_destroy(Shard *e);
int shard_set_eigen(Shard *e, const double *eval, const double *evec, const double *ivec);
int shard_set_frequencies(Shard *e, const double *freqs);
int shard_set_category_rates(Shard *e, const double *rates, const double *proportions);

int shard_create(const phyamd_config *cfg, Shard **out) {
	if (!cfg || !out) return fail(PHYAMD_EINVAL, "null argument");
	*out = nullptr;
	if (cfg->tip_count < 2) return fail(PHYAMD_EINVAL, "tip_count must be >= 2 (got %d)", cfg->tip_count);
	if (cfg->pattern_count < 1) return fail(PHYAMD_EINVAL, "pattern_count must be >= 1 (got %d)", cfg->pattern_count);
	if (cfg->category_count < 1) return fail(PHYAMD_EINVAL, "category_count must be >= 1 (got %d)", cfg->category_count);
	if (cfg->state_count != 4 && cfg->state_count != 20 && cfg->state_count != 60 && cfg->state_count != 61)
		return fail(PHYAMD_EUNSUPPORTED, "state_count %d: kernels are built for 4, 20, 60 and 61 states", cfg->state_count);
	if (cfg->rescale < 0 || cfg->rescale > 2) return fail(PHYAMD_EINVAL, "rescale must be PHYAMD_RESCALE_*");
	if (cfg->category_count > MAX_WAVES)
		return fail(PHYAMD_EUNSUPPORTED, "category_count %d exceeds %d (one wave per category)", cfg->category_count, MAX_WAVES);
	int ndev = 0;
	HIP_TRY(hipGetDeviceCount(&ndev));
	if (ndev == 0) return fail(PHYAMD_EDEVICE, "no HIP device visible");
	Shard *e = new Shard();
	e->cfg = *cfg;
	e->mem.cap = cfg->max_device_bytes;
	e->T = cfg->tip_count;
	e->N = 2 * e->T - 1;
	e->P = e->Ptot = cfg->pattern_count;
	e->S = cfg->state_count;
	e->C = cfg->category_count;
	if (cfg->device >= 0) e->device = cfg->device;
	else if (hipGetDevice(&e->device) != hipSuccess) e->device = 0;
	if (e->device >= ndev) {
		delete e;
		return fail(PHYAMD_EINVAL, "device %d out of range (%d visible)", cfg->device, ndev);
	}
	auto bail = [&](int rc) {
		shard_destroy(e);
		return rc;
	};
	int rc;
	{
		hipError_t err = hipSetDevice(e->device);
		if (err != hipSuccess) return bail(fail(PHYAMD_EDEVICE, "hipSetDevice(%d): %s", e->device, hipGetErrorString(err)));
	}
	if ((rc = choose_tiles(e, false))) return bail(rc);
	if (cfg->stream) e->stream = (hipStream_t)cfg->stream;
	else {
		hipError_t err = hipStreamCreateWithFlags(&e->stream, hipStreamNonBlocking);
		if (err != hipSuccess) return bail(fail(PHYAMD_EDEVICE, "hipStreamCreate: %s", hipGetErrorString(err)));
		e->own_stream = true;
	}
	e->scaling_on = cfg->rescale == PHYAMD_RESCALE_ALWAYS;
	if (const char *env = std::getenv("PHYAMD_FUSE")) e->fusion_enabled = std::atoi(env) != 0;
	if (const char *env = std::getenv("PHYAMD_WALK")) e->walk_enabled = std::atoi(env) != 0;
	if (const char *env = std::getenv("PHYAMD_GEN_FUSION")) e->generic_fusion = std::atoi(env) != 0;
	if (const char *env = std::getenv("PHYAMD_XCD_MAP")) e->xcd_map = std::atoi(env) != 0;
	if (const char *env = std::getenv("PHYAMD_SCALE_EXP2")) e->exp2_on = std::atoi(env) != 0;
	if (const char *env = std::getenv("PHYAMD_STREAM_TFORM")) e->tform_on = std::atoi(env) != 0;
	if (const char *env = std::getenv("PHYAMD_LOWER_PARK2")) e->lower_park2_on = std::atoi(env) != 0;
	e->generic = e->S != 4;
	e->tip_set.assign(e->T, 0);
	e->tip_empty.assign(e->T, 0);
	e->mem.spare = &e->batch_mem;
	e->batch_max_patterns = BATCH_MAX_PATTERNS;
	if (const char *env = std::getenv("PHYAMD_BATCH_MAX_PATTERNS")) e->batch_max_patterns = std::atoi(env);
	if (const char *env = std::getenv("PHYAMD_BATCH_TRACE")) e->batch_trace = std::atoi(env) != 0;
	e->explicit_host.assign(e->N, 0);
	const size_t msz = (size_t)e->N * e->C * e->S * e->S;
	if (e->generic && ((rc = e->d_tipsets.ensure(256)) || (rc = e->d_imgs.ensure(((size_t)e->N * e->C + 2) * gen_image_doubles(e))))) return bail(rc);
	if (e->S == 20 && GenFuse<2>::QP) {
		if ((rc = e->d_qp_mats.ensure((size_t)e->T * e->C * e->S * e->S)) || (rc = e->d_qp_imgs.ensure((size_t)e->T * e->C * gen_image_doubles(e)))) return bail(rc);
	}
	if ((rc = e->d_mats.ensure(msz)) || (rc = e->d_dmats.ensure(msz)) || (rc = e->d_model.ensure((size_t)e->S + 2 * e->S * e->S)) ||
	    (rc = e->d_Q.ensure((size_t)e->S * e->S)))
		return bail(rc);
	if (!e->generic && (rc = e->d_tiptab.ensure((size_t)e->T * e->C * 64 + (size_t)e->N * 6))) return bail(rc);
	if ((rc = e->d_freqs.ensure(e->S)) || (rc = e->d_rates.ensure(e->C)) || (rc = e->d_props.ensure(e->C)) || (rc = e->d_lengths.ensure(e->N)) ||
	    (rc = e->d_result.ensure((size_t)1 + e->N * e->C + 2 * PHYAMD_MAX_PARAMETERS)) || (rc = e->d_explicit.ensure(e->N)) ||
	    (rc = e->d_row_valid.ensure((size_t)e->N * e->C)))
		return bail(rc);
	{
		hipError_t err = hipHostMalloc(reinterpret_cast<void **>(&e->h_result), sizeof(double) * ((size_t)2 + e->N * e->C + 2 * PHYAMD_MAX_PARAMETERS), hipHostMallocDefault);
		if (err != hipSuccess) return bail(fail(PHYAMD_EDEVICE, "hipHostMalloc: %s", hipGetErrorString(err)));
		err = hipMemsetAsync(e->d_explicit, 0, e->N, e->stream);
		if (err == hipSuccess) err = hipStreamSynchronize(e->stream);
		if (err != hipSuccess) return bail(fail(PHYAMD_EDEVICE, "memset: %s", hipGetErrorString(err)));
		for (auto &ev : e->ev) {
			err = hipEventCreate(&ev);
			if (err != hipSuccess) return bail(fail(PHYAMD_EDEVICE, "hipEventCreate: %s", hipGetErrorString(err)));
		}
	}
	if ((rc = allocate_pattern_storage(e))) return bail(rc);
	*out = e;
	return PHYAMD_OK;
}

void shard_destroy(Shard *e) {
	if (!e) return;
	(void)hipSetDevice(e->device);
	if (e->stream) (void)hipStreamSynchronize(e->stream);
	if (e->h_result) (void)hipHostFree(e->h_result);
	if (e->h_lengths) (void)hipHostFree(e->h_lengths);
	if (e->ev_lengths) (void)hipEventDestroy(e->ev_lengths);
	if (e->ev_check) (void)hipEventDestroy(e->ev_check);
	for (auto &ev : e->ev)
		if (ev) (void)hipEventDestroy(ev);
	if (e->own_stream && e->stream) (void)hipStreamDestroy(e->stream);
	delete e;
}

#define CHECK_ENGINE(e) \
	if (!(e)) return fail(PHYAMD_EINVAL, "null engine")

int shard_set_tip_states(Shard *e, int tip, const uint8_t *states) {
	CHECK_ENGINE(e);
	if (tip < 0 || tip >= e->T || !states) return fail(PHYAMD_EINVAL, "bad tip %d or null states", tip);
	int rc;
	if ((rc = bind_device(e))) return rc;
	std::vector<uint8_t> mask(e->Ptot);
	if (e->generic)
		for (int k = 0; k < e->Ptot; k++) mask[k] = states[k] < e->S ? states[k] : (uint8_t)e->S;
	else
		for (int k = 0; k < e->Ptot; k++) mask[k] = states[k] < 4 ? (uint8_t)(1u << states[k]) : (uint8_t)0xF;
	HIP_TRY(hipMemcpyAsync(tip_row(e, tip), mask.data(), e->Ptot, hipMemcpyHostToDevice, e->stream));
	HIP_TRY(hipStreamSynchronize(e->stream));
	e->tip_set[tip] = 1;
	e->tip_empty[tip] = 0;
	input_changed(e, Input::TipData);
	return PHYAMD_OK;
}

int shard_set_tip_partials(Shard *e, int tip, const double *partials) {
	CHECK_ENGINE(e);
	if (tip < 0 || tip >= e->T || !partials) return fail(PHYAMD_EINVAL, "bad tip %d or null partials", tip);
	int rc;
	if ((rc = bind_device(e))) return rc;
	std::vector<uint8_t> mask(e->Ptot);
	if (e->generic) {
		const int S = e->S;
		for (int k = 0; k < e->Ptot; k++) {
			int ones = 0, last = -1;
			unsigned long long members = 0;
			for (int s = 0; s < S; s++) {
				const double v = partials[(size_t)k * S + s];
				if (v == 1.0) ones++, last = s, members |= 1ull << s;
				else if (v != 0.0) return fail(PHYAMD_EUNSUPPORTED, "tip %d pattern %d: only 0/1 tip partials are built", tip, k);
			}
			if (ones == 1) mask[k] = (uint8_t)last;
			else if (ones == S) mask[k] = (uint8_t)S;
			else {
				size_t q = std::find(e->tipsets_host.begin(), e->tipsets_host.end(), members) - e->tipsets_host.begin();
				if (q == e->tipsets_host.size()) {
					if ((int)q + S + 1 > 255) return fail(PHYAMD_EUNSUPPORTED, "tip %d pattern %d: more than %d distinct ambiguity sets", tip, k, 255 - S);
					e->tipsets_host.push_back(members);
				}
				mask[k] = (uint8_t)(S + 1 + q);
			}
		}
		if (e->tipsets_uploaded != e->tipsets_host.size()) {
			HIP_TRY(hipMemcpyAsync(e->d_tipsets, e->tipsets_host.data(), e->tipsets_host.size() * sizeof(unsigned long long), hipMemcpyHostToDevice, e->stream));
			e->tipsets_uploaded = e->tipsets_host.size();
		}
	} else {
		for (int k = 0; k < e->Ptot; k++) {
			unsigned m = 0;
			for (int s = 0; s < 4; s++) {
				const double v = partials[(size_t)k * 4 + s];
				if (v == 1.0) m |= 1u << s;
				else if (v != 0.0)
					return fail(PHYAMD_EUNSUPPORTED, "tip %d pattern %d: tip partials other than 0/1 ambiguity masks are not built in this revision", tip, k);
			}
			mask[k] = (uint8_t)m;
		}
		e->tip_empty[tip] = std::find(mask.begin(), mask.end(), (uint8_t)0) != mask.end();
	}
	HIP_TRY(hipMemcpyAsync(tip_row(e, tip), mask.data(), e->Ptot, hipMemcpyHostToDevice, e->stream));
	HIP_TRY(hipStreamSynchronize(e->stream));
	e->tip_set[tip] = 1;
	input_changed(e, Input::TipData);
	return PHYAMD_OK;
}

int shard_set_pattern_weights(Shard *e, const double *weights) {
	CHECK_ENGINE(e);
	if (!weights) return fail(PHYAMD_EINVAL, "null weights");
	int rc;
	if ((rc = bind_device(e))) return rc;
	HIP_TRY(hipMemcpyAsync(e->tiles > 1 ? e->d_weights_all : e->d_weights, weights, sizeof(double) * e->Ptot, hipMemcpyHostToDevice, e->stream));
	HIP_TRY(hipStreamSynchronize(e->stream));
	e->have_weights = true;
	input_changed(e, Input::PatternWeights);
	return PHYAMD_OK;
}

int shard_set_topology(Shard *e, const int32_t *left, const int32_t *right, int root) {
	CHECK_ENGINE(e);
	if (!left || !right) return fail(PHYAMD_EINVAL, "null topology arrays");
	int rc;
	if ((rc = bind_device(e))) return rc;
	e->batch_mem.release_all();
	lowers_discarded(e);
	std::vector<int32_t> old_l = e->left, old_r = e->right;
	const int old_root = e->root;
	e->left.assign(left, left + e->N);
	e->right.assign(right, right + e->N);
	e->root = root;
	const bool had_topology = e->have_topology;
	auto roll_back = [&](int code) {
		const std::string why = g_last_error;
		e->left = old_l;
		e->right = old_r;
		e->root = old_root;
// ... 1725 lines not shown
```

### physher_amd/csrc/phyamd_walk4s.inc

```

enum { HK_TIP = 0, HK_CHERRY = 1, HK_CHERRY_TIP = 2 };
enum { SU_CARRY = 0, SU_LDS = 1, SU_U = 2, SU_ROOT = 3 };

struct StreamOp {
	int32_t flags;
	int32_t parent;
	int32_t slot_parent, slot_left, slot_right;
	int32_t nx_mask_word;
	int32_t nx_a, nx_b;
	int32_t lnode, la[10];
	int32_t rnode, ra[10];
	int32_t nx_u;
	int32_t wsh;
};
static_assert(sizeof(StreamOp) == 128, "one StreamOp = 32 dwords");

struct StreamDesc {
	int32_t flags;
	int32_t parent, lnode, rnode;
	int32_t lm[5], rm[5];
	int64_t nx_words;
	int64_t nx_a, nx_b, nx_u;
	int64_t st_left, st_right;
	int32_t wsh;
	int32_t pad[5];
};
static_assert(sizeof(StreamDesc) == 128 && offsetof(StreamDesc, nx_words) == 56, "one StreamDesc = 32 dwords");

struct StreamChunk {
	int32_t mask_word, mask_words, a, b, u, same_row, pad[2];
};

constexpr int OPBLK_BYTES = 2048, OPBLK_LEFT = 64, OPBLK_RIGHT = 1024, OPTIP_BYTES = 160;

__global__ __launch_bounds__(256) void k_build_mask_stream(int rows, int P, size_t mstride, const int *__restrict__ row_entries, const uint8_t *__restrict__ tipmask,
                                                           uint32_t *__restrict__ mstream, int *__restrict__ flags) {
	const size_t k = (size_t)blockIdx.x * 256 + threadIdx.x;
	if (k >= mstride) return;
	bool bad = false, amb = false;
	for (int w = blockIdx.y; w < rows; w += gridDim.y) {
		uint32_t v = 0;
		for (int j = 0; j < 8; j++) {
			const int ent = row_entries[w * 8 + j];
			if (ent < 0) continue;
			const int t = ent & 0xFFFFF, pos = (ent >> 20) & 31, fpos = (ent >> 25) & 31;
			const uint32_t m = (k < (size_t)P ? tipmask[(size_t)t * P + k] : 0xFu) & 0xFu;
			const uint32_t code = m == 1 ? 0 : m == 2 ? 1 : m == 4 ? 2 : m == 8 ? 3 : (m == 15 || m == 0) ? 4 : m == 3 ? 5 : m < 8 ? m + 1 : m;
			bad |= m == 0;
			if (code >= 5) {
				amb = true;
				v |= 1u << fpos;
			}
			v |= code << pos;
		}
		mstream[(size_t)w * mstride + k] = v;
	}
	if (bad || amb) atomicOr(flags, (bad ? 1 : 0) | (amb ? 2 : 0));
}

__global__ __launch_bounds__(64) void k_op_tables(int nops, int C, const int *__restrict__ op_tips, const int *__restrict__ op_deep, const int *__restrict__ site_tab,
                                                  const double *__restrict__ mats, const double *__restrict__ Qs, double *__restrict__ optab) {
	const int op = blockIdx.x, c = blockIdx.y, t = threadIdx.x;
	double *blk = optab + ((size_t)c * nops + op) * (OPBLK_BYTES / 8);
	if (t < 16) reinterpret_cast<int *>(blk)[t] = site_tab[op * 16 + t];
	const int deep = op_deep[op];
	for (int e = t; e < 2 * 120; e += 64) {
		const int side = e / 120, f = e % 120;
		const bool dp = (deep >> side) & 1;
		const int slot = dp ? f / 20 : f / 40, g = dp ? f % 20 : f % 40;
		const bool qrow = !dp && g >= 20;
		const int row = (g % 20) / 4, i = g % 4;
		const int tip = op_tips[op * 12 + side * 6 + slot];
		double v = 0.0;
		if (tip >= 0) {
			const double *M = mats + ((size_t)tip * C + c) * 16;
			double col[4];
			for (int r = 0; r < 4; r++) col[r] = row < 4 ? M[r * 4 + row] : ((M[r * 4] + M[r * 4 + 1]) + (M[r * 4 + 2] + M[r * 4 + 3]));
			v = !qrow ? col[i] : Qs ? Qs[i * 4] * col[0] + Qs[i * 4 + 1] * col[1] + Qs[i * 4 + 2] * col[2] + Qs[i * 4 + 3] * col[3] : 0.0;
		}
		blk[(side ? OPBLK_RIGHT : OPBLK_LEFT) / 8 + f] = v;
	}
}

typedef const __attribute__((address_space(3))) char *lds_cptr;
typedef __attribute__((address_space(3))) dv2 lds_dv2;

__device__ __forceinline__ d4 lds_read4(lds_cptr p) {
	const lds_dv2 *q = (const lds_dv2 *)p;
	const dv2 lo = q[0], hi = q[1];
	return d4{lo.x, lo.y, hi.x, hi.y};
}

struct SX {
	const char *__restrict__ mats_c;
	lds_cptr tb;
	__device__ __forceinline__ cptr M(int off) const { return opaque(as_const(reinterpret_cast<const double *>(mats_c + (unsigned)off))); }
	template <int J>
	static __device__ __forceinline__ unsigned row(unsigned w) {
		return J == 0 ? (w << 4) & 0xE0u : J == 1 ? w & 0xE0u : (w >> (4 * J - 4)) & 0xE0u;
	}
	bool amb = false;
	template <int J>
	__device__ __forceinline__ d4 tip_rows(unsigned rows_off, unsigned w) const {
		const unsigned code = (w >> (4 * J + 1)) & 15u;
		const unsigned tbu = (unsigned)(uintptr_t)tb;
		const lds_cptr rows = (lds_cptr)(uintptr_t)tbu + rows_off;
		d4 v = lds_read4((lds_cptr)(uintptr_t)(tbu | ((amb && code >= 5u) ? 0u : row<J>(w))) + rows_off);
		if (amb) {
			if (code >= 5u) {
				const unsigned m = (unsigned)(0xEDCBA97653ull >> (4u * (code - 5u))) & 15u;
				v = d4{0., 0., 0., 0.};
#pragma unroll
				for (int st = 0; st < 4; st++)
					if (m >> st & 1u) {
						const d4 r = lds_read4(rows + 32 * st);
						v = d4{v.x + r.x, v.y + r.y, v.z + r.z, v.w + r.w};
					}
			}
		}
		return v;
	}
	template <int SIDE, int SLOT>
	__device__ __forceinline__ d4 deep_tip(unsigned w) const {
		return tip_rows<SLOT>((SIDE ? OPBLK_RIGHT : OPBLK_LEFT) + SLOT * OPTIP_BYTES, w);
	}
	template <int SIDE, int SLOT>
	__device__ __forceinline__ d4 site_tip(unsigned w) const {
		return tip_rows<SLOT>((SIDE ? OPBLK_RIGHT : OPBLK_LEFT) + SLOT * 2 * OPTIP_BYTES, w);
	}
	template <int SIDE, int SLOT>
	__device__ __forceinline__ d4 site_tip_q(unsigned w) const {
		return tip_rows<SLOT>((SIDE ? OPBLK_RIGHT : OPBLK_LEFT) + SLOT * 2 * OPTIP_BYTES + OPTIP_BYTES, w);
	}
};

template <int SIDE, int SB>
__device__ __forceinline__ d4 s_half(const SX &x, int hk, int mnode, int minner, unsigned w) {
	if (hk == HK_TIP) return x.deep_tip<SIDE, SB>(w);
	d4 p = mul4(x.deep_tip<SIDE, SB>(w), x.deep_tip<SIDE, SB + 1>(w));
	if (hk == HK_CHERRY_TIP) p = mul4(matvec4_opt<false>(x.M(minner), p), x.deep_tip<SIDE, SB + 2>(w));
	return matvec4_opt<false>(x.M(mnode), p);
}

template <bool WEIGHTED>
struct SiteSum {
	double acc0, acc1, acc2;
	double sel0, sel1, sel2, sel3;
	cptr Q;
	double wq = 1.0;
	template <int A, int R, bool FIRST>
	__device__ __forceinline__ void put(double num) {
		const double s = R == 0 ? sel0 : R == 1 ? sel1 : R == 2 ? sel2 : sel3;
		double &acc = A == 0 ? acc0 : A == 1 ? acc1 : acc2;
		acc = __builtin_amdgcn_mfma_f64_4x4x4f64(s, WEIGHTED ? wq * num : num, FIRST ? 0.0 : acc, 0, 0, 0);
	}
	template <int A, int R, bool FIRST = false>
	__device__ __forceinline__ void add(const d4 &u, const d4 &b) {
		put<A, R, FIRST>(dot4(u, matvec4_opt<false>(opaque(Q), b)));
	}
	template <int A, int R, bool FIRST = false>
	__device__ __forceinline__ void add_tip(const d4 &u, const d4 &qb) {
		put<A, R, FIRST>(dot4(u, qb));
	}
};

template <int SIDE, bool KEEP_BN>
__device__ __forceinline__ d4 s_fringe_message(const SX &x, int kind, int node, int inner, unsigned w, d4 &bn) {
	d4 p = mul4(x.site_tip<SIDE, 0>(w), x.site_tip<SIDE, 1>(w));
	if (kind == CH_CHERRY_TIP) {
		const d4 inner_message = matvec4_opt<false>(x.M(inner), p);
		if (KEEP_BN) bn = inner_message;
		p = mul4(inner_message, x.site_tip<SIDE, 2>(w));
	}
	return matvec4_opt<false>(x.M(node), p);
}

template <int SIDE, bool FIRST2, bool KEEP_BN, typename SS>
__device__ __forceinline__ void s_descend(const SX &x, SS &ss, int kind, int node, int inner, const d4 &u, unsigned w, const d4 &bn_kept) {
	d4 a2 = matvec4_opt<false>(x.M(node), u);
	if (kind == CH_CHERRY_TIP) {
		const d4 bn = KEEP_BN ? bn_kept : matvec4_opt<false>(x.M(inner), mul4(x.site_tip<SIDE, 0>(w), x.site_tip<SIDE, 1>(w)));
		const d4 un = mul4(a2, x.site_tip<SIDE, 2>(w));
		ss.template add<SIDE, 3>(un, bn);
		ss.template add_tip<2, SIDE, FIRST2>(mul4(a2, bn), x.site_tip_q<SIDE, 2>(w));
		a2 = matvec4_opt<false>(x.M(inner), un);
	}
	ss.template add_tip<SIDE, 1>(mul4(a2, x.site_tip<SIDE, 1>(w)), x.site_tip_q<SIDE, 0>(w));
	ss.template add_tip<SIDE, 2>(mul4(a2, x.site_tip<SIDE, 0>(w)), x.site_tip_q<SIDE, 1>(w));
}

__device__ __forceinline__ double dpp_f64(double old, double src, const int ctrl, const int bank) {
	const int lo = __double2loint(src), hi = __double2hiint(src), olo = __double2loint(old), ohi = __double2hiint(old);
	int rlo, rhi;
	switch (ctrl * 16 + bank) {
#define PHYAMD_DPP_CASE(CT, BK)                                              \
	case (CT) * 16 + (BK):                                                   \
		rlo = __builtin_amdgcn_update_dpp(olo, lo, CT, 0xF, BK, false);      \
		rhi = __builtin_amdgcn_update_dpp(ohi, hi, CT, 0xF, BK, false);      \
		break;
		PHYAMD_DPP_CASE(0x140, 0x3)
		PHYAMD_DPP_CASE(0x140, 0xC)
		PHYAMD_DPP_CASE(0x140, 0xF)
		PHYAMD_DPP_CASE(0x141, 0x5)
		PHYAMD_DPP_CASE(0x141, 0xA)
		PHYAMD_DPP_CASE(0x141, 0xF)
		PHYAMD_DPP_CASE(0xE4, 0xC)
		PHYAMD_DPP_CASE(0xE4, 0xA)
		PHYAMD_DPP_CASE(0x1B, 0xF)
		PHYAMD_DPP_CASE(0xB1, 0xF)
#undef PHYAMD_DPP_CASE
		default: rlo = lo; rhi = hi;
	}
	return __hiloint2double(rhi, rlo);
}

template <bool THREE>
__device__ __forceinline__ double fold_sites(double acc0, double acc1, double acc2) {
	const double y01 = dpp_f64(dpp_f64(0.0, acc0, 0x140, 0x3), acc1, 0x140, 0xC);
	const double x01 = dpp_f64(acc0, acc1, 0xE4, 0xC);
	const double s01 = x01 + y01;
	double z;
	if (THREE) {
		const double s2 = acc2 + dpp_f64(0.0, acc2, 0x140, 0xF);
		const double y = dpp_f64(dpp_f64(0.0, s01, 0x141, 0x5), s2, 0x141, 0xA);
		const double xk = dpp_f64(s01, s2, 0xE4, 0xA);
		z = xk + y;
	} else
		z = s01 + dpp_f64(0.0, s01, 0x141, 0xF);
	z += dpp_f64(0.0, z, 0x1B, 0xF);
	z += dpp_f64(0.0, z, 0xB1, 0xF);
	return z;
}

__device__ __forceinline__ int exp2_rescale(d4 &v) {
	const double m = max4(v);
	if (!(m < SCALING_THRESHOLD) || !(m > 0.0)) return 0;
	const int e = ((__double2hiint(m) >> 20) & 0x7FF) - 1023;
	v = d4{__builtin_amdgcn_ldexp(v.x, -e), __builtin_amdgcn_ldexp(v.y, -e), __builtin_amdgcn_ldexp(v.z, -e), __builtin_amdgcn_ldexp(v.w, -e)};
	return e;
}

constexpr int STREAM_MIN_WAVES = 4;
constexpr int STREAM_MIN_WAVES_SCALE = 3;

__device__ __forceinline__ void dma_piece(const char *gsrc, lds_cptr dst) {
	__builtin_amdgcn_global_load_lds((const __attribute__((address_space(1))) void *)gsrc, (__attribute__((address_space(3))) void *)dst, 16, 0, 0);
}

typedef double dv4 __attribute__((ext_vector_type(4)));
__device__ __forceinline__ d4 prefetch4(const char *base, unsigned lane_off, bool nt) {
	dv2 lo, hi;
	if (nt) asm volatile("global_load_dwordx4 %0, %2, %3 nt\n\tglobal_load_dwordx4 %1, %2, %3 offset:16 nt" : "=&v"(lo), "=&v"(hi) : "v"(lane_off), "s"(base) : "memory");
	else asm volatile("global_load_dwordx4 %0, %2, %3\n\tglobal_load_dwordx4 %1, %2, %3 offset:16" : "=&v"(lo), "=&v"(hi) : "v"(lane_off), "s"(base) : "memory");
	return d4{lo.x, lo.y, hi.x, hi.y};
}
__device__ __forceinline__ unsigned prefetch1(const char *base, unsigned lane_off) {
	unsigned w;
	asm volatile("global_load_dword %0, %1, %2" : "=v"(w) : "v"(lane_off), "s"(base) : "memory");
	return w;
}

constexpr int STREAM_PARK_SLOTS = 2, STREAM_PARK_BYTES = 2 * WAVE * 16;
constexpr int STREAM_LDS_PER_WAVE = STREAM_PARK_SLOTS * STREAM_PARK_BYTES + 2 * OPBLK_BYTES;

constexpr int STREAM_WAVES = 4;

__device__ __forceinline__ unsigned xcd_position(unsigned x, unsigned n, int on) {
	if (!on) return x;
	const unsigned r = x & 7u, q = n >> 3, m = n & 7u;
	return r * q + (r < m ? r : m) + (x >> 3);
}

__device__ __forceinline__ void any_value(d4 &v) { asm volatile("" : "=v"(v.x), "=v"(v.y), "=v"(v.z), "=v"(v.w)); }
__device__ __forceinline__ d4 own_registers(const d4 &v) {
	d4 r;
	asm volatile("v_mov_b64 %0, %1" : "=v"(r.x) : "v"(v.x));
	asm volatile("v_mov_b64 %0, %1" : "=v"(r.y) : "v"(v.y));
	asm volatile("v_mov_b64 %0, %1" : "=v"(r.z) : "v"(v.z));
	asm volatile("v_mov_b64 %0, %1" : "=v"(r.w) : "v"(v.w));
	return r;
}
template <bool FOLD, int SCALE, bool AMBIG = false, bool TF = false>
__global__ __launch_bounds__(STREAM_WAVES *WAVE, (SCALE || AMBIG) ? STREAM_MIN_WAVES_SCALE : STREAM_MIN_WAVES) void k_upper4_stream(
    const StreamDesc *__restrict__ ops, const StreamChunk *__restrict__ chunks, const int *__restrict__ chunk_off, int chunk_base, int nops, int P, int C, int nb,
    const uint32_t *__restrict__ mstream, size_t mstride, const double *__restrict__ lower, double *__restrict__ upper, const double *__restrict__ mats,
    const char *__restrict__ optab, const double *__restrict__ Q, const double *__restrict__ freqs, const double *__restrict__ w_over_L,
    double *__restrict__ gslab, int R, const double *__restrict__ props, const double *__restrict__ weights, int xcd_map, const int *__restrict__ lexp,
    int *__restrict__ uexp, const int *__restrict__ Eroot) {
	extern __shared__ double sh[];
	constexpr bool KEEP_BN = !SCALE && !AMBIG;
	constexpr bool XCH = SCALE == 1, EXP2 = SCALE == 2;
	const int lane = threadIdx.x, wv = __builtin_amdgcn_readfirstlane(threadIdx.y);
	const unsigned vx = XCH ? blockIdx.x : xcd_position(blockIdx.x, gridDim.x, xcd_map);
	const int c = XCH ? wv : vx % C, blk = XCH ? (int)blockIdx.x : (int)(vx / C) * STREAM_WAVES + wv;
	if (blk >= nb) return;
	const size_t plane = (size_t)P * 4;
	const int k0 = blk * WAVE + lane;
	const bool valid = k0 < P;
	const unsigned k = valid ? k0 : P - 1;
	const unsigned poff = k * 32u;
	const unsigned moff = (unsigned)k0 * 4u;
	const lds_cptr wave_lds = (lds_cptr)sh + (size_t)wv * STREAM_LDS_PER_WAVE;
	const lds_cptr blocks = wave_lds + STREAM_PARK_SLOTS * STREAM_PARK_BYTES;
	SX x{reinterpret_cast<const char *>(mats + (size_t)c * 16), blocks};
	const double wl = SCALE ? 1.0 : (valid ? w_over_L[k] : 0.0);
	const double wk = XCH ? (valid ? weights[k] : 0.0) : EXP2 ? (valid ? w_over_L[k] : 0.0) : 0.0;
	const double pc = XCH ? props[c] : 0.0;
	const int eroot = EXP2 ? Eroot[k] : 0;
	double *const xbase = sh + (size_t)blockDim.y * (STREAM_LDS_PER_WAVE / 8);
	const int xsz = blockDim.y * WAVE;
	int *const pexp = reinterpret_cast<int *>(xbase) + ((size_t)wv * STREAM_PARK_SLOTS) * WAVE + lane;
	const char *const lexp_c = EXP2 ? reinterpret_cast<const char *>(lexp) + (size_t)c * P * 4 : nullptr;
	char *const uexp_c = EXP2 ? reinterpret_cast<char *>(uexp) + (size_t)c * P * 4 : nullptr;
	const unsigned eoff = k * 4u;
	SiteSum<SCALE != 0> ss;
	ss.Q = as_const(Q);
	ss.sel0 = (lane & 3) == 0 ? 1.0 : 0.0;
	ss.sel1 = (lane & 3) == 1 ? 1.0 : 0.0;
	ss.sel2 = (lane & 3) == 2 ? 1.0 : 0.0;
	ss.sel3 = (lane & 3) == 3 ? 1.0 : 0.0;
	const int n16 = lane & 15, r4 = lane >> 4;
	const unsigned cid4 = (unsigned)(n16 == 0 ? r4 : n16 == 8 ? 4 + r4 : n16 == 4 ? 8 + r4 : 15) * 4u;
	char *const slab = reinterpret_cast<char *>(gslab + ((size_t)blk * C + c) * R);
	__attribute__((address_space(3))) dv2 *park = (__attribute__((address_space(3))) dv2 *)wave_lds + lane;
	const int chunk = chunk_base + blockIdx.y;
	const int op_begin = chunk_off[chunk], op_end = chunk_off[chunk + 1];
	const char *const optab_c = optab + (size_t)c * nops * OPBLK_BYTES + lane * 16;

	const char *const lower_c = reinterpret_cast<const char *>(lower + (size_t)c * plane);
	char *const upper_c = reinterpret_cast<char *>(upper + (size_t)c * plane);
	const char *const mstream_b = reinterpret_cast<const char *>(mstream);
	const size_t mrow = mstride * 4;
	constexpr bool ASM_PREFETCH = true;
	auto lower_at = [&](int64_t off) -> d4 {
		return ASM_PREFETCH ? prefetch4(lower_c + off, poff, true) : load4_stream(reinterpret_cast<const double *>(lower_c + off + poff));
	};
	auto upper_at = [&](int64_t off) -> d4 { return ASM_PREFETCH ? prefetch4(upper_c + off, poff, false) : load4(reinterpret_cast<const double *>(upper_c + off + poff)); };
	auto store_upper_at = [&](int64_t off, const d4 &v) { store4(reinterpret_cast<double *>(upper_c + off + poff), v); };
	auto word_at = [&](int64_t off) -> unsigned { return ASM_PREFETCH ? prefetch1(mstream_b + off, moff) : *reinterpret_cast<const unsigned *>(mstream_b + off + moff); };
	auto fetch_lower = [&](int core) -> d4 { return load4_stream(reinterpret_cast<const double *>(reinterpret_cast<const char *>(lower + ((size_t)core * C + c) * plane) + poff)); };
	auto fetch_upper = [&](int slot) -> d4 { return load4(reinterpret_cast<const double *>(reinterpret_cast<const char *>(upper + ((size_t)slot * C + c) * plane) + poff)); };
	auto fetch_word = [&](int w) -> unsigned { return *reinterpret_cast<const unsigned *>(reinterpret_cast<const char *>(mstream + (size_t)w * mstride) + moff); };
	auto fetch_block = [&](int op_index, bool two) {
		const char *src = optab_c + (size_t)op_index * OPBLK_BYTES;
		const lds_cptr dst = blocks + (op_index & 1) * OPBLK_BYTES;
		dma_piece(src, dst);
		if (two) dma_piece(src + 1024, dst + 1024);
	};

	unsigned w0 = 0, w1 = 0;
	d4 A = d4{1., 1., 1., 1.}, B = A, U = A;
	int eA = 0, eB = 0, eU = 0;
	if (op_begin < op_end) {
		const StreamChunk ch = chunks[chunk];
		fetch_block(op_begin, true);
		if (ch.mask_words > 0) w0 = fetch_word(ch.mask_word);
		if (ch.mask_words > 1) w1 = fetch_word(ch.mask_word + (ch.same_row ? 0 : 1));
		if (ch.a != -1) A = fetch_lower(ch.a);
		if (ch.b != -1) B = fetch_lower(ch.b);
		if (ch.u != -1) U = fetch_upper(ch.u);
		if (EXP2) {
			if (ch.a != -1) eA = *reinterpret_cast<const int *>(lexp_c + (size_t)ch.a * C * P * 4 + eoff);
			if (ch.b != -1) eB = *reinterpret_cast<const int *>(lexp_c + (size_t)ch.b * C * P * 4 + eoff);
			if (ch.u != -1) eU = *reinterpret_cast<const int *>(uexp_c + (size_t)ch.u * C * P * 4 + eoff);
		}
	}
	d4 ul = A;
	int e_ul = 0;
	double prev_tot = 0.0;
	int prev_off = -1;
#pragma unroll 1
	for (int i = op_begin; i < op_end; i++) {
		StreamDesc op;
		{
			typedef const __attribute__((address_space(4))) int32_t *ciptr;
			const ciptr raw = (ciptr)(ops + i);
			int32_t *dst = reinterpret_cast<int32_t *>(&op);
#pragma unroll
			for (int j = 0; j < 27; j++) dst[j] = raw[j];
		}
		asm volatile("s_waitcnt vmcnt(0)" ::: "memory");
		if (prev_off >= 0) *reinterpret_cast<double *>(slab + (unsigned)prev_off) = prev_tot;
		const int fl = op.flags;
		const int kl = fl & 7, kr = (fl >> 3) & 7;
		const int usrc = (fl >> 9) & 7, pk = (fl >> 12) & 3, nxw = (fl >> 14) & 3;
		x.tb = blocks + (i & 1) * OPBLK_BYTES;
		const int soff = *(const __attribute__((address_space(3))) int *)(x.tb + cid4);
		const unsigned g0 = w0 >> (op.wsh & 31), g1 = w1 >> ((op.wsh >> 5) & 31);
		const unsigned wL = g0, wR = (kl != CH_CORE) ? g1 : g0;
		if (AMBIG) x.amb = __any((int)((g0 | (kl != CH_CORE && kr != CH_CORE ? g1 : 0u)) & 1u)) != 0;
		d4 a;
		int ea = 0;
		if (usrc == SU_CARRY) {
			a = matvec4_opt<false>(x.M(op.parent), ul);
			ea = e_ul;
		} else if (usrc == SU_LDS) {
			const int ps = STREAM_PARK_SLOTS > 1 ? ((fl >> 7) & 1) * (STREAM_PARK_BYTES / 16) : 0;
			const dv2 lo = park[ps], hi = park[ps + WAVE];
			a = matvec4_opt<false>(x.M(op.parent), d4{lo.x, lo.y, hi.x, hi.y});
			if (EXP2) ea = pexp[(STREAM_PARK_SLOTS > 1 ? (fl >> 7) & 1 : 0) * WAVE];
		} else if (usrc == SU_U) {
			ea = eU;
			a = matvec4_opt<false>(x.M(op.parent), U);
			if (!SCALE && !valid) a = d4{0., 0., 0., 0.};
		}
		else a = FOLD ? d4{wl * freqs[0], wl * freqs[1], wl * freqs[2], wl * freqs[3]} : d4{wl, wl, wl, wl};
		d4 bl, br, bnl, bnr;
		if (KEEP_BN) {
			any_value(bnl);
			any_value(bnr);
		}
		if (kl == CH_CORE) bl = TF ? own_registers(A) : matvec4_opt<false>(x.M(op.lnode), A);
		else if (kl == CH_TIP) bl = x.site_tip<0, 0>(wL);
		else if (kl == CH_DEEP)
			bl = matvec4_opt<false>(x.M(op.lnode), mul4(s_half<0, 0>(x, (fl >> 16) & 3, op.lm[0], op.lm[1], wL), s_half<0, 3>(x, (fl >> 18) & 3, op.lm[2], op.lm[3], wL)));
		else bl = s_fringe_message<0, KEEP_BN>(x, kl, op.lnode, op.lm[4], wL, bnl);
		if (kr == CH_CORE) br = TF ? own_registers(B) : matvec4_opt<false>(x.M(op.rnode), B);
		else if (kr == CH_TIP) br = x.site_tip<1, 0>(wR);
		else if (kr == CH_DEEP)
			br = matvec4_opt<false>(x.M(op.rnode), mul4(s_half<1, 0>(x, (fl >> 20) & 3, op.rm[0], op.rm[1], wR), s_half<1, 3>(x, (fl >> 22) & 3, op.rm[2], op.rm[3], wR)));
		else br = s_fringe_message<1, KEEP_BN>(x, kr, op.rnode, op.rm[4], wR, bnr);
		const int e_bl = EXP2 && kl == CH_CORE ? eA : 0, e_br = EXP2 && kr == CH_CORE ? eB : 0;
		__builtin_amdgcn_s_setprio(3);
		unsigned nw0 = 0, nw1 = 0;
		if (i + 1 < op_end) fetch_block(i + 1, (fl >> 24) & 1);
		if (nxw > 0) nw0 = word_at(op.nx_words);
		if (nxw > 1) nw1 = word_at(op.nx_words + ((fl >> 25) & 1 ? (int64_t)0 : (int64_t)mrow));
		if (fl & (1 << 26)) A = lower_at(op.nx_a);
		if (fl & (1 << 27)) B = lower_at(op.nx_b);
		if (fl & (1 << 28)) U = upper_at(op.nx_u);
		if (EXP2) {
			if (fl & (1 << 26)) eA = *reinterpret_cast<const int *>(lexp_c + (op.nx_a >> 3) + eoff);
			if (fl & (1 << 27)) eB = *reinterpret_cast<const int *>(lexp_c + (op.nx_b >> 3) + eoff);
			if (fl & (1 << 28)) eU = *reinterpret_cast<const int *>(uexp_c + (op.nx_u >> 3) + eoff);
		}
		__builtin_amdgcn_s_setprio(0);
		ul = mul4(a, br);
		d4 ur = mul4(a, bl);
		d4 ul_terms = ul, ur_terms = ur;
		int e_l = 0, e_r = 0;
		if (EXP2) {
			ss.wq = __builtin_amdgcn_ldexp(wk, ea + e_bl + e_br - eroot);
			e_l = ea + e_br + exp2_rescale(ul);
			e_r = ea + e_bl + exp2_rescale(ur);
		}
		if (XCH) {
			const double den = dot4(FOLD ? a : d4{freqs[0] * a.x, freqs[1] * a.y, freqs[2] * a.z, freqs[3] * a.w}, mul4(bl, br));
			double *xb = xbase + (size_t)(i & 1) * 2 * xsz;
			int2 *xm = reinterpret_cast<int2 *>(xb + xsz);
			xb[wv * WAVE + lane] = pc * den;
			xm[wv * WAVE + lane] = int2{__double2hiint(max4(ul)) + 1, __double2hiint(max4(ur)) + 1};
			lds_barrier();
			double D = 0.0;
			int mlh = 0, mrh = 0;
			for (int cc = 0; cc < C; cc++) {
				D += xb[cc * WAVE + lane];
				const int2 m2 = xm[cc * WAVE + lane];
				mlh = max(mlh, m2.x);
				mrh = max(mrh, m2.y);
			}
			ss.wq = wk / D;
			const double ml = __hiloint2double(mlh, 0), mr = __hiloint2double(mrh, 0);
			if (ml < SCALING_THRESHOLD) ul = d4{ul.x / ml, ul.y / ml, ul.z / ml, ul.w / ml};
			if (mr < SCALING_THRESHOLD) ur = d4{ur.x / mr, ur.y / mr, ur.z / mr, ur.w / mr};
		}
		if (pk) {
			const d4 &v = pk == 1 ? ul : ur;
			const int ps = STREAM_PARK_SLOTS > 1 ? ((fl >> 6) & 1) * (STREAM_PARK_BYTES / 16) : 0;
			park[ps] = dv2{v.x, v.y};
			park[ps + WAVE] = dv2{v.z, v.w};
			if (EXP2) pexp[(STREAM_PARK_SLOTS > 1 ? (fl >> 6) & 1 : 0) * WAVE] = pk == 1 ? e_l : e_r;
		}
		if ((fl & (1 << 29)) && valid) store_upper_at(op.st_left, ul);
		if ((fl & (1 << 30)) && valid) store_upper_at(op.st_right, ur);
		if (EXP2) {
			if ((fl & (1 << 29)) && valid) *reinterpret_cast<int *>(uexp_c + (op.st_left >> 3) + eoff) = e_l;
			if ((fl & (1 << 30)) && valid) *reinterpret_cast<int *>(uexp_c + (op.st_right >> 3) + eoff) = e_r;
		}
		if (kl == CH_TIP) ss.template add_tip<0, 0, true>(ul_terms, x.site_tip_q<0, 0>(wL));
		else ss.template add<0, 0, true>(ul_terms, bl);
		if (kr == CH_TIP) ss.template add_tip<1, 0, true>(ur_terms, x.site_tip_q<1, 0>(wR));
		else ss.template add<1, 0, true>(ur_terms, br);
		if (kl == CH_CHERRY_TIP) {
			s_descend<0, true, KEEP_BN>(x, ss, CH_CHERRY_TIP, op.lnode, op.lm[4], ul_terms, wL, bnl);
			if (kr >= CH_CHERRY) s_descend<1, false, KEEP_BN>(x, ss, kr, op.rnode, op.rm[4], ur_terms, wR, bnr);
			prev_tot = fold_sites<true>(ss.acc0, ss.acc1, ss.acc2);
		} else if (kr == CH_CHERRY_TIP) {
			if (kl == CH_CHERRY) s_descend<0, false, KEEP_BN>(x, ss, CH_CHERRY, op.lnode, op.lm[4], ul_terms, wL, bnl);
			s_descend<1, true, KEEP_BN>(x, ss, CH_CHERRY_TIP, op.rnode, op.rm[4], ur_terms, wR, bnr);
			prev_tot = fold_sites<true>(ss.acc0, ss.acc1, ss.acc2);
		} else {
			if (kl == CH_CHERRY) s_descend<0, false, KEEP_BN>(x, ss, CH_CHERRY, op.lnode, op.lm[4], ul_terms, wL, bnl);
			if (kr == CH_CHERRY) s_descend<1, false, KEEP_BN>(x, ss, CH_CHERRY, op.rnode, op.rm[4], ur_terms, wR, bnr);
			prev_tot = fold_sites<false>(ss.acc0, ss.acc1, 0.0);
		}
		prev_off = soff;
		w0 = nw0;
		w1 = nw1;
		e_ul = e_l;
	}
	if (prev_off >= 0) *reinterpret_cast<double *>(slab + (unsigned)prev_off) = prev_tot;
}

struct LowerDesc {
	int32_t flags;
	int32_t nx_block;
	int32_t lnode, rnode, lm[5], rm[5];
	int64_t nx_words;
	int64_t store;
	int64_t mem_l, mem_r;
	int32_t wsh;
	int32_t self;
	int64_t ls_store, ls_l, ls_r;
	int32_t pad[2];
};
static_assert(sizeof(LowerDesc) == 128 && offsetof(LowerDesc, nx_words) == 56, "one LowerDesc = 32 dwords");
struct LowerChunk {
	int32_t block, pieces, mask_rows, slot;
	int64_t words;
};

constexpr int LSTREAM_MIN_WAVES = 5;
constexpr int lstream_park_slots(bool ambig) { return ambig ? 1 : 2; }
constexpr int LSTREAM_LDS_PER_WAVE = 2 * OPBLK_BYTES + 5 * WAVE * 4 + WAVE * 32;

__device__ __forceinline__ void dma_dword(const char *gsrc, lds_cptr dst) {
	__builtin_amdgcn_global_load_lds((const __attribute__((address_space(1))) void *)gsrc, (__attribute__((address_space(3))) void *)dst, 4, 0, 0);
}

template <bool AMBIG, int SCALE, bool TF = false>
__global__ __launch_bounds__(STREAM_WAVES *WAVE, SCALE == 1 ? 4 : LSTREAM_MIN_WAVES) void k_lower4_stream(
    const LowerDesc *__restrict__ ops, const LowerChunk *__restrict__ chunks, const int *__restrict__ chunk_off, int chunk_base, int nblocks, int P, int C, int nb,
    const uint32_t *__restrict__ mstream, size_t mstride, double *__restrict__ lower, const double *__restrict__ mats, const char *__restrict__ optab,
    const double *__restrict__ freqs, const double *__restrict__ props, double *__restrict__ Lc, int with_root, double *__restrict__ lscale, int xcd_map,
    int *__restrict__ Ec) {
	extern __shared__ double sh[];
	constexpr bool XCH = SCALE == 1, EXP2 = SCALE == 2, PARK2 = lstream_park_slots(AMBIG) > 1;
	const int lane = threadIdx.x, wv = __builtin_amdgcn_readfirstlane(threadIdx.y);
	const unsigned vx = XCH ? blockIdx.x : xcd_position(blockIdx.x, gridDim.x, xcd_map);
	const int c = XCH ? wv : vx % C, blk = XCH ? (int)blockIdx.x : (int)(vx / C) * STREAM_WAVES + wv;
	if (blk >= nb) return;
	const size_t plane = (size_t)P * 4;
	const int k0 = blk * WAVE + lane;
	const bool valid = k0 < P;
	const unsigned k = valid ? k0 : P - 1;
	const unsigned poff = k * 32u, moff = (unsigned)k0 * 4u;
	const lds_cptr blocks = (lds_cptr)sh + (size_t)wv * LSTREAM_LDS_PER_WAVE;
	const lds_cptr wrows = blocks + 2 * OPBLK_BYTES;
	SX x{reinterpret_cast<const char *>(mats + (size_t)c * 16), blocks};
	const int chunk = chunk_base + blockIdx.y;
	const int op_begin = chunk_off[chunk], op_end = chunk_off[chunk + 1];
	const char *const optab_c = optab + (size_t)c * nblocks * OPBLK_BYTES + lane * 16;
	char *const lower_c = reinterpret_cast<char *>(lower + (size_t)c * plane);
	const char *const mstream_b = reinterpret_cast<const char *>(mstream) + moff;
	const size_t mrow = mstride * 4;
	const char *const hot = optab + (size_t)c * nblocks * OPBLK_BYTES + lane * 4;
	auto request_words = [&](int64_t off, int count, int slot) {
		dma_dword(count > 0 ? mstream_b + off : hot, wrows + (count > 0 ? slot : 4) * (WAVE * 4));
		dma_dword(count > 1 ? mstream_b + off + mrow : hot, wrows + (count > 1 ? ((slot + 1) & 3) : 4) * (WAVE * 4));
	};
	auto request_block = [&](int parity, int block, int pieces) {
		const char *src = optab_c + (size_t)block * OPBLK_BYTES;
		const lds_cptr dst = blocks + parity * OPBLK_BYTES;
		if (pieces & 1) dma_piece(src, dst);
		else dma_dword(hot, wrows + 4 * (WAVE * 4));
		if (pieces & 2) dma_piece(src + 1024, dst + 1024);
		else dma_dword(hot, wrows + 4 * (WAVE * 4));
	};
	if (op_begin < op_end) {
		const LowerChunk ch = chunks[chunk];
		request_block(op_begin & 1, ch.block, ch.pieces);
		request_words(ch.words, ch.mask_rows, ch.slot);
	}
	const lds_cptr stage = wrows + 5 * WAVE * 4;
	const bool valid_lo = blk * WAVE + (lane >> 1) < P, valid_hi = blk * WAVE + 32 + (lane >> 1) < P, full_block = (blk + 1) * WAVE <= P;
	auto store_result = [&](int64_t off, const d4 &v) {
		__attribute__((address_space(3))) dv2 *w = (__attribute__((address_space(3))) dv2 *)(stage + lane * 32);
		w[0] = dv2{v.x, v.y};
// ... 164 lines not shown
```

Before: 36.45.

## Precompute per-op cherry message tables and read them from LDS in pre-order walk

```diff
diff --git a/include/physher_amd.h b/include/physher_amd.h
--- a/include/physher_amd.h
+++ b/include/physher_amd.h
@@ -108,6 +108,8 @@
 int phyamd_get_node_matrices(phyamd_engine *e, int node, int derivative, double *out );
 int phyamd_post_order_parks(int32_t tip_count, const int32_t *left , const int32_t *right, int32_t root, int32_t second_slot,
                             int32_t *out , int32_t capacity);
+int phyamd_pre_order_cherry_tables(int32_t tip_count, const int32_t *left , const int32_t *right, int32_t root,
+                                   int32_t *out , int32_t capacity);
 int phyamd_is_rescaling(phyamd_engine *e);
 int phyamd_set_rescaling(phyamd_engine *e, int policy);
 int phyamd_set_keep_partials(phyamd_engine *e, int on);
diff --git a/physher_amd/_lib.py b/physher_amd/_lib.py
--- a/physher_amd/_lib.py
+++ b/physher_amd/_lib.py
@@ -96,6 +96,7 @@
     ("phyamd_get_partials", C.c_int, [_P, C.c_int, C.c_int, _P]),
     ("phyamd_get_node_matrices", C.c_int, [_P, C.c_int, C.c_int, _P]),
     ("phyamd_post_order_parks", C.c_int, [C.c_int32, _P, _P, C.c_int32, C.c_int32, _P, C.c_int32]),
+    ("phyamd_pre_order_cherry_tables", C.c_int, [C.c_int32, _P, _P, C.c_int32, _P, C.c_int32]),
     ("phyamd_is_rescaling", C.c_int, [_P]),
     ("phyamd_set_rescaling", C.c_int, [_P, C.c_int]),
     ("phyamd_set_keep_partials", C.c_int, [_P, C.c_int]),
diff --git a/physher_amd/csrc/phyamd_abi.inc b/physher_amd/csrc/phyamd_abi.inc
--- a/physher_amd/csrc/phyamd_abi.inc
+++ b/physher_amd/csrc/phyamd_abi.inc
@@ -718,6 +718,31 @@
 	return (int)ops.size();
 }
 
+int phyamd_pre_order_cherry_tables(int32_t tip_count, const int32_t *left, const int32_t *right, int32_t root, int32_t *out, int32_t capacity) {
+	if (tip_count < 2) return fail(PHYAMD_EINVAL, "tip_count must be >= 2 (got %d)", tip_count);
+	if (!left || !right) return fail(PHYAMD_EINVAL, "null left or right");
+	if (capacity < 0 || (capacity > 0 && !out)) return fail(PHYAMD_EINVAL, "null out with capacity %d", capacity);
+	std::unique_ptr<Shard> e(new Shard());
+	e->T = tip_count;
+	e->N = 2 * e->T - 1;
+	e->S = 4;
+	e->C = 1;
+	e->P = e->Ptot = 1;
+	e->root = root;
+	e->left.assign(left, left + e->N);
+	e->right.assign(right, right + e->N);
+	int rc;
+	if ((rc = build_schedule(e.get()))) return rc;
+	build_stream_ops(e.get());
+	const int n = (int)e->stream_ops.size();
+	for (int i = 0; i < n && i < capacity; i++) {
+		const int *info = &e->stream_cherry_info[(size_t)i * 2], *d = &e->stream_ctab_desc[(size_t)i * 4];
+		const int32_t rec[6] = {e->stream_ops[i].parent, info[0], info[1], d[0], d[1], d[2]};
+		std::memcpy(out + (size_t)i * 6, rec, sizeof(rec));
+	}
+	return n;
+}
+
 int phyamd_is_rescaling(phyamd_engine *g) {
 	CHECK_GROUP(g);
 	int any = 0;
diff --git a/physher_amd/csrc/phyamd_launch.inc b/physher_amd/csrc/phyamd_launch.inc
--- a/physher_amd/csrc/phyamd_launch.inc
+++ b/physher_amd/csrc/phyamd_launch.inc
@@ -349,6 +349,10 @@
 	const bool capped = e->cfg.max_device_bytes > 0;
 	int rc = ensure_mask_stream(e);
 	if (!rc) rc = ensure_optab(e);
+	if (!rc && !lower && e->cherry_tables_on && e->d_ctab.ensure((size_t)std::max<size_t>(1, e->stream_ops.size()) * e->C * CTAB_BYTES)) {
+		e->cherry_tables_on = false;
+		rc = upload_schedule(e);
+	}
 	if (!rc && lower) rc = e->d_Lc.ensure((size_t)e->C * e->P);
 	if (rc == PHYAMD_ENOMEM && capped) {
 		(lower ? e->lower_stream_capped : e->upper_stream_capped) = true;
@@ -417,10 +421,16 @@
 	const bool exp2 = v.scale == 2, tf = v.tf;
 	if (exp2 && (rc = e->d_uexp.ensure(std::max<size_t>(1, upper_slots_held(e)) * e->C * e->P))) return rc;
 	const int waves = SCALE && !exp2 ? e->C : STREAM_WAVES;
-	const size_t lds = (size_t)STREAM_LDS_PER_WAVE * waves + (exp2 ? (size_t)waves * STREAM_PARK_SLOTS * WAVE * sizeof(int) : SCALE ? (size_t)4 * e->C * WAVE * sizeof(double) : 0);
+	const bool ctabs = e->cherry_tables_on && v.scale == 0 && !e->stream_ambiguous;
+	if (ctabs && e->d_ctab.size() < (size_t)nops * e->C * CTAB_BYTES) return fail(PHYAMD_EDEVICE, "streamed walk: the cherry tables have no array");
+	const size_t lds = (size_t)(STREAM_LDS_PER_WAVE + (ctabs ? STREAM_LDS_CTABS : 0)) * waves +
+	                   (exp2 ? (size_t)waves * STREAM_PARK_SLOTS * WAVE * sizeof(int) : SCALE ? (size_t)4 * e->C * WAVE * sizeof(double) : 0);
 	const dim3 grid_x(SCALE && !exp2 ? (unsigned)nb : (unsigned)((nb + STREAM_WAVES - 1) / STREAM_WAVES) * e->C), block(WAVE, waves);
 	hipLaunchKernelGGL(k_op_tables, dim3(nops, e->C), dim3(64), 0, e->stream, nops, e->C, (const int *)e->d_stream_op_tips, (const int *)e->d_stream_op_deep,
 	                   (const int *)e->d_stream_site_tab, e->d_mats, FOLD ? e->d_Q : e->d_Qpi, reinterpret_cast<double *>(e->d_optab.get()));
+	if (ctabs)
+		hipLaunchKernelGGL(k_cherry_tables, dim3(nops, e->C), dim3(64), 0, e->stream, nops, e->C, reinterpret_cast<const int4 *>(e->d_stream_ctab_desc.get()),
+		                   (const double *)e->d_mats, reinterpret_cast<double *>(e->d_ctab.get()));
 	const int subtrees = (int)e->walk_chunk_off.size() - 2;
 	for (int phase = 0; phase < (subtrees > 0 ? 2 : 1); phase++) {
 		const bool amb = e->stream_ambiguous;
@@ -431,7 +441,8 @@
 		hipLaunchKernelGGL(kernel, dim3(grid_x.x, phase ? subtrees : 1), block, lds, e->stream, (const StreamDesc *)e->d_stream_ops, (const StreamChunk *)e->d_stream_chunks,
 		                   (const int *)e->d_walk_chunk_off, phase, nops, e->P, e->C, nb, (const uint32_t *)e->d_mstream, e->mstride, (const double *)e->d_lower, e->d_upper,
 		                   (const double *)e->d_mats, (const char *)e->d_optab, (const double *)(FOLD ? e->d_Q : e->d_Qpi), (const double *)e->d_freqs, (const double *)e->d_wl,
-		                   e->d_gslab, R, (const double *)e->d_props, (const double *)e->d_weights, e->xcd_map, (const int *)e->d_lexp, e->d_uexp, (const int *)e->d_Eroot);
+		                   e->d_gslab, R, (const double *)e->d_props, (const double *)e->d_weights, e->xcd_map, (const int *)e->d_lexp, e->d_uexp, (const int *)e->d_Eroot,
+		                   ctabs ? (const char *)e->d_ctab : (const char *)nullptr);
 	}
 	HIP_TRY(hipGetLastError());
 	e->prof.upper_launches = subtrees > 0 ? 2 : 1;
diff --git a/physher_amd/csrc/phyamd_schedule.inc b/physher_amd/csrc/phyamd_schedule.inc
--- a/physher_amd/csrc/phyamd_schedule.inc
+++ b/physher_amd/csrc/phyamd_schedule.inc
@@ -221,6 +221,8 @@
 	e->stream_op_deep.assign(n, 0);
 	e->stream_qnode.clear();
 	e->stream_words = 0;
+	e->stream_ctab_desc.assign((size_t)n * 4, -1);
+	e->stream_cherry_info.assign((size_t)n * 2, 0);
 	if (n == 0) return;
 	std::vector<NodeOp> src = e->walk_chunk_ops;
 	std::vector<char> chunk_start(n + 1, 0);
@@ -309,6 +311,23 @@
 				}
 			}
 			for (int j = 0; j < 6; j++) e->stream_op_tips[(size_t)i * 12 + 6 * side + j] = tips[j];
+			auto candidate = [&](int pos, int mnode, int t0, int t1) {
+				int *info = &e->stream_cherry_info[(size_t)i * 2];
+				info[0]++;
+				if (!e->cherry_tables_on) return;
+				info[1] = pos;
+				const int rec[4] = {mnode, t0, t1, -1};
+				std::copy(rec, rec + 4, &e->stream_ctab_desc[(size_t)i * 4]);
+			};
+			if (kind == CH_CHERRY) candidate(1 + side, node, a[0], a[1]);
+			else if (kind == CH_CHERRY_TIP) candidate(1 + side, a[3], a[0], a[1]);
+			else if (kind == CH_DEEP)
+				for (int h = 0; h < 2; h++) {
+					const int32_t *q = a + 5 * h;
+					const int hk = h ? e->deep_host[node].kind_right : e->deep_host[node].kind_left;
+					if (hk == CH_CHERRY) candidate(3 + 2 * side + h, q[0], q[1], q[2]);
+					else if (hk == CH_CHERRY_TIP) candidate(3 + 2 * side + h, q[4], q[1], q[2]);
+				}
 			if (kind != CH_CORE) {
 				int row, shift;
 				packer.add(tips, row, shift);
@@ -333,6 +352,7 @@
 		}
 		fl |= usrc << 9;
 		s.flags = fl;
+		s.wsh |= e->stream_cherry_info[(size_t)i * 2 + 1] << 10;
 		const int sites[10] = {o.left, o.kind_left >= CH_CHERRY ? o.lt0 : -1, o.kind_left >= CH_CHERRY ? o.lt1 : -1, o.kind_left == CH_CHERRY_TIP ? o.linner : -1,
 		                       o.right, o.kind_right >= CH_CHERRY ? o.rt0 : -1, o.kind_right >= CH_CHERRY ? o.rt1 : -1, o.kind_right == CH_CHERRY_TIP ? o.rinner : -1,
 		                       o.kind_left == CH_CHERRY_TIP ? o.lt2 : -1, o.kind_right == CH_CHERRY_TIP ? o.rt2 : -1};
@@ -348,7 +368,7 @@
 	for (int k = 0; k < chunks; k++) {
 		const int b = e->walk_chunk_off[k], en = e->walk_chunk_off[k + 1];
 		StreamChunk ch{-1, 0, -1, -1, -1, 0, {0, 0}};
-		if (b < en) ch = StreamChunk{first_word[b], words[b], want_a[b], want_b[b], want_u[b], same_row[b], {0, 0}};
+		if (b < en) ch = StreamChunk{first_word[b], words[b], want_a[b], want_b[b], want_u[b], same_row[b], {e->stream_cherry_info[(size_t)b * 2 + 1] != 0, 0}};
 		e->stream_chunks.push_back(ch);
 		for (int i = b; i < en; i++) {
 			StreamOp &s = e->stream_ops[i];
@@ -357,6 +377,7 @@
 			s.flags |= (last ? 0 : words[i + 1]) << 14;
 			s.flags |= (!last && src[i + 1].kind_right != CH_CORE ? 1 : 0) << 24;
 			s.flags |= (!last && same_row[i + 1] ? 1 : 0) << 25;
+			s.flags |= (!last && e->stream_cherry_info[(size_t)(i + 1) * 2 + 1] != 0 ? 1 : 0) << 8;
 			s.nx_a = last ? -1 : want_a[i + 1];
 			s.nx_b = last ? -1 : want_b[i + 1];
 			s.nx_u = last ? -1 : want_u[i + 1];
@@ -816,8 +837,9 @@
 			build_lower_stream_ops(e);
 			if ((rc = e->d_stream_ops.ensure(e->N)) || (rc = e->d_stream_chunks.ensure((size_t)e->N + 2)) || (rc = e->d_stream_row_entries.ensure((size_t)e->N * 32)) ||
 			    (rc = e->d_stream_site_tab.ensure((size_t)e->N * 16)) || (rc = e->d_stream_qnode.ensure(e->N)) || (rc = e->d_stream_op_tips.ensure((size_t)e->N * 12)) ||
-			    (rc = e->d_stream_flag.ensure(1)) || (rc = e->d_stream_op_deep.ensure(e->N)))
+			    (rc = e->d_stream_flag.ensure(1)) || (rc = e->d_stream_op_deep.ensure(e->N)) || (rc = e->d_stream_ctab_desc.ensure((size_t)e->N * 4)))
 				return rc;
+			HIP_TRY(hipMemcpyAsync(e->d_stream_ctab_desc, e->stream_ctab_desc.data(), e->stream_ctab_desc.size() * sizeof(int), hipMemcpyHostToDevice, e->stream));
 			HIP_TRY(hipMemcpyAsync(e->d_stream_op_tips, e->stream_op_tips.data(), e->stream_op_tips.size() * sizeof(int), hipMemcpyHostToDevice, e->stream));
 			HIP_TRY(hipMemcpyAsync(e->d_stream_op_deep, e->stream_op_deep.data(), e->stream_op_deep.size() * sizeof(int), hipMemcpyHostToDevice, e->stream));
 			HIP_TRY(hipMemcpyAsync(e->d_stream_ops, e->stream_desc.data(), e->stream_desc.size() * sizeof(StreamDesc), hipMemcpyHostToDevice, e->stream));
diff --git a/physher_amd/csrc/phyamd_shard.inc b/physher_amd/csrc/phyamd_shard.inc
--- a/physher_amd/csrc/phyamd_shard.inc
+++ b/physher_amd/csrc/phyamd_shard.inc
@@ -91,6 +91,11 @@
 	std::vector<int> stream_op_deep;
 	DeviceArray<int> d_stream_op_tips{&mem}, d_stream_flag{&mem}, d_stream_op_deep{&mem};
 	DeviceArray<char> d_optab{&mem};
+	bool cherry_tables_on = true;
+	std::vector<int> stream_ctab_desc;
+	std::vector<int> stream_cherry_info;
+	DeviceArray<int> d_stream_ctab_desc{&mem};
+	DeviceArray<char> d_ctab{&mem};
 	bool stream_ambiguous = false;
 	bool stream_unsupported = false;
 	int stream_words = 0, stream_R = 0;
diff --git a/physher_amd/csrc/phyamd_shard_api.inc b/physher_amd/csrc/phyamd_shard_api.inc
--- a/physher_amd/csrc/phyamd_shard_api.inc
+++ b/physher_amd/csrc/phyamd_shard_api.inc
@@ -162,6 +162,8 @@
 	if (const char *env = std::getenv("PHYAMD_SCALE_EXP2")) e->exp2_on = std::atoi(env) != 0;
 	if (const char *env = std::getenv("PHYAMD_STREAM_TFORM")) e->tform_on = std::atoi(env) != 0;
 	if (const char *env = std::getenv("PHYAMD_LOWER_PARK2")) e->lower_park2_on = std::atoi(env) != 0;
+	if (const char *env = std::getenv("PHYAMD_CHERRY_TABLES")) e->cherry_tables_on = std::atoi(env) != 0;
+	if (cfg->max_device_bytes > 0) e->cherry_tables_on = false;
 	e->generic = e->S != 4;
 	e->tip_set.assign(e->T, 0);
 	e->tip_empty.assign(e->T, 0);
diff --git a/physher_amd/csrc/phyamd_walk4s.inc b/physher_amd/csrc/phyamd_walk4s.inc
--- a/physher_amd/csrc/phyamd_walk4s.inc
+++ b/physher_amd/csrc/phyamd_walk4s.inc
@@ -32,6 +32,9 @@
 };
 
 constexpr int OPBLK_BYTES = 2048, OPBLK_LEFT = 64, OPBLK_RIGHT = 1024, OPTIP_BYTES = 160;
+
+enum { CTAB_NONE = 0, CTAB_LEFT = 1, CTAB_RIGHT = 2, CTAB_LEFT_H0 = 3, CTAB_LEFT_H1 = 4, CTAB_RIGHT_H0 = 5, CTAB_RIGHT_H1 = 6 };
+constexpr int CTAB_BYTES = 1024;
 
 __global__ __launch_bounds__(256) void k_build_mask_stream(int rows, int P, size_t mstride, const int *__restrict__ row_entries, const uint8_t *__restrict__ tipmask,
                                                            uint32_t *__restrict__ mstream, int *__restrict__ flags) {
@@ -82,6 +85,20 @@
 	}
 }
 
+__global__ __launch_bounds__(64) void k_cherry_tables(int nops, int C, const int4 *__restrict__ desc, const double *__restrict__ mats, double *__restrict__ ctab) {
+	const int op = blockIdx.x, c = blockIdx.y, t = threadIdx.x;
+	const int4 d = desc[op];
+	if (d.x < 0 || t >= 25) return;
+	auto tip_row = [&](int tip, int s) {
+		const double *M = mats + ((size_t)tip * C + c) * 16;
+		double col[4];
+		for (int r = 0; r < 4; r++) col[r] = s < 4 ? M[r * 4 + s] : ((M[r * 4] + M[r * 4 + 1]) + (M[r * 4 + 2] + M[r * 4 + 3]));
+		return d4{col[0], col[1], col[2], col[3]};
+	};
+	const d4 m = matvec4_opt<false>(as_const(mats + ((size_t)d.x * C + c) * 16), mul4(tip_row(d.y, t / 5), tip_row(d.z, t % 5)));
+	store4(ctab + ((size_t)c * nops + op) * (CTAB_BYTES / 8) + t * 4, m);
+}
+
 typedef const __attribute__((address_space(3))) char *lds_cptr;
 typedef __attribute__((address_space(3))) dv2 lds_dv2;
 
@@ -100,6 +117,11 @@
 		return J == 0 ? (w << 4) & 0xE0u : J == 1 ? w & 0xE0u : (w >> (4 * J - 4)) & 0xE0u;
 	}
 	bool amb = false;
+	lds_cptr ct = nullptr;
+	template <int J>
+	__device__ __forceinline__ d4 cherry_row(unsigned w) const {
+		return lds_read4(ct + (((w >> (4 * J + 1)) & 7u) * 160u + row<J + 1>(w)));
+	}
 	template <int J>
 	__device__ __forceinline__ d4 tip_rows(unsigned rows_off, unsigned w) const {
 		const unsigned code = (w >> (4 * J + 1)) & 15u;
@@ -135,8 +157,13 @@
 };
 
 template <int SIDE, int SB>
-__device__ __forceinline__ d4 s_half(const SX &x, int hk, int mnode, int minner, unsigned w) {
+__device__ __forceinline__ d4 s_half(const SX &x, int hk, int mnode, int minner, unsigned w, int tpos = CTAB_NONE) {
 	if (hk == HK_TIP) return x.deep_tip<SIDE, SB>(w);
+	if (tpos == CTAB_LEFT_H0 + 2 * SIDE + SB / 3) {
+		const d4 m = x.cherry_row<SB>(w);
+		if (hk != HK_CHERRY_TIP) return m;
+		return matvec4_opt<false>(x.M(mnode), mul4(m, x.deep_tip<SIDE, SB + 2>(w)));
+	}
 	d4 p = mul4(x.deep_tip<SIDE, SB>(w), x.deep_tip<SIDE, SB + 1>(w));
 	if (hk == HK_CHERRY_TIP) p = mul4(matvec4_opt<false>(x.M(minner), p), x.deep_tip<SIDE, SB + 2>(w));
 	return matvec4_opt<false>(x.M(mnode), p);
@@ -165,7 +192,13 @@
 };
 
 template <int SIDE, bool KEEP_BN>
-__device__ __forceinline__ d4 s_fringe_message(const SX &x, int kind, int node, int inner, unsigned w, d4 &bn) {
+__device__ __forceinline__ d4 s_fringe_message(const SX &x, int kind, int node, int inner, unsigned w, d4 &bn, int tpos = CTAB_NONE) {
+	if (tpos == CTAB_LEFT + SIDE) {
+		const d4 m = x.cherry_row<0>(w);
+		if (kind != CH_CHERRY_TIP) return m;
+		if (KEEP_BN) bn = m;
+		return matvec4_opt<false>(x.M(node), mul4(m, x.site_tip<SIDE, 2>(w)));
+	}
 	d4 p = mul4(x.site_tip<SIDE, 0>(w), x.site_tip<SIDE, 1>(w));
 	if (kind == CH_CHERRY_TIP) {
 		const d4 inner_message = matvec4_opt<false>(x.M(inner), p);
@@ -262,6 +295,7 @@
 
 constexpr int STREAM_PARK_SLOTS = 2, STREAM_PARK_BYTES = 2 * WAVE * 16;
 constexpr int STREAM_LDS_PER_WAVE = STREAM_PARK_SLOTS * STREAM_PARK_BYTES + 2 * OPBLK_BYTES;
+constexpr int STREAM_LDS_CTABS = 2 * CTAB_BYTES;
 
 constexpr int STREAM_WAVES = 4;
 
@@ -286,9 +320,11 @@
     const uint32_t *__restrict__ mstream, size_t mstride, const double *__restrict__ lower, double *__restrict__ upper, const double *__restrict__ mats,
     const char *__restrict__ optab, const double *__restrict__ Q, const double *__restrict__ freqs, const double *__restrict__ w_over_L,
     double *__restrict__ gslab, int R, const double *__restrict__ props, const double *__restrict__ weights, int xcd_map, const int *__restrict__ lexp,
-    int *__restrict__ uexp, const int *__restrict__ Eroot) {
+    int *__restrict__ uexp, const int *__restrict__ Eroot, const char *__restrict__ ctab) {
 	extern __shared__ double sh[];
 	constexpr bool KEEP_BN = !SCALE && !AMBIG;
+	constexpr bool TABLES = !SCALE && !AMBIG;
+	const bool tables = TABLES && ctab != nullptr;
 	constexpr bool XCH = SCALE == 1, EXP2 = SCALE == 2;
 	const int lane = threadIdx.x, wv = __builtin_amdgcn_readfirstlane(threadIdx.y);
 	const unsigned vx = XCH ? blockIdx.x : xcd_position(blockIdx.x, gridDim.x, xcd_map);
@@ -300,8 +336,9 @@
 	const unsigned k = valid ? k0 : P - 1;
 	const unsigned poff = k * 32u;
 	const unsigned moff = (unsigned)k0 * 4u;
-	const lds_cptr wave_lds = (lds_cptr)sh + (size_t)wv * STREAM_LDS_PER_WAVE;
+	const lds_cptr wave_lds = (lds_cptr)sh + (size_t)wv * (STREAM_LDS_PER_WAVE + (tables ? STREAM_LDS_CTABS : 0));
 	const lds_cptr blocks = wave_lds + STREAM_PARK_SLOTS * STREAM_PARK_BYTES;
+	const lds_cptr ctabs = blocks + 2 * OPBLK_BYTES;
 	SX x{reinterpret_cast<const char *>(mats + (size_t)c * 16), blocks};
 	const double wl = SCALE ? 1.0 : (valid ? w_over_L[k] : 0.0);
 	const double wk = XCH ? (valid ? weights[k] : 0.0) : EXP2 ? (valid ? w_over_L[k] : 0.0) : 0.0;
@@ -347,6 +384,8 @@
 		dma_piece(src, dst);
 		if (two) dma_piece(src + 1024, dst + 1024);
 	};
+	const char *const ctab_c = ctab + (size_t)c * nops * CTAB_BYTES + lane * 16;
+	auto fetch_ctab = [&](int op_index) { dma_piece(ctab_c + (size_t)op_index * CTAB_BYTES, ctabs + (op_index & 1) * CTAB_BYTES); };
 
 	unsigned w0 = 0, w1 = 0;
 	d4 A = d4{1., 1., 1., 1.}, B = A, U = A;
@@ -354,6 +393,7 @@
 	if (op_begin < op_end) {
 		const StreamChunk ch = chunks[chunk];
 		fetch_block(op_begin, true);
+		if (TABLES && ch.pad[0]) fetch_ctab(op_begin);
 		if (ch.mask_words > 0) w0 = fetch_word(ch.mask_word);
 		if (ch.mask_words > 1) w1 = fetch_word(ch.mask_word + (ch.same_row ? 0 : 1));
 		if (ch.a != -1) A = fetch_lower(ch.a);
@@ -385,6 +425,8 @@
 		const int kl = fl & 7, kr = (fl >> 3) & 7;
 		const int usrc = (fl >> 9) & 7, pk = (fl >> 12) & 3, nxw = (fl >> 14) & 3;
 		x.tb = blocks + (i & 1) * OPBLK_BYTES;
+		const int tpos = TABLES ? (op.wsh >> 10) & 7 : 0;
+		if (TABLES) x.ct = ctabs + (i & 1) * CTAB_BYTES;
 		const int soff = *(const __attribute__((address_space(3))) int *)(x.tb + cid4);
 		const unsigned g0 = w0 >> (op.wsh & 31), g1 = w1 >> ((op.wsh >> 5) & 31);
 		const unsigned wL = g0, wR = (kl != CH_CORE) ? g1 : g0;
@@ -413,17 +455,18 @@
 		if (kl == CH_CORE) bl = TF ? own_registers(A) : matvec4_opt<false>(x.M(op.lnode), A);
 		else if (kl == CH_TIP) bl = x.site_tip<0, 0>(wL);
 		else if (kl == CH_DEEP)
-			bl = matvec4_opt<false>(x.M(op.lnode), mul4(s_half<0, 0>(x, (fl >> 16) & 3, op.lm[0], op.lm[1], wL), s_half<0, 3>(x, (fl >> 18) & 3, op.lm[2], op.lm[3], wL)));
-		else bl = s_fringe_message<0, KEEP_BN>(x, kl, op.lnode, op.lm[4], wL, bnl);
+			bl = matvec4_opt<false>(x.M(op.lnode), mul4(s_half<0, 0>(x, (fl >> 16) & 3, op.lm[0], op.lm[1], wL, tpos), s_half<0, 3>(x, (fl >> 18) & 3, op.lm[2], op.lm[3], wL, tpos)));
+		else bl = s_fringe_message<0, KEEP_BN>(x, kl, op.lnode, op.lm[4], wL, bnl, tpos);
 		if (kr == CH_CORE) br = TF ? own_registers(B) : matvec4_opt<false>(x.M(op.rnode), B);
 		else if (kr == CH_TIP) br = x.site_tip<1, 0>(wR);
 		else if (kr == CH_DEEP)
-			br = matvec4_opt<false>(x.M(op.rnode), mul4(s_half<1, 0>(x, (fl >> 20) & 3, op.rm[0], op.rm[1], wR), s_half<1, 3>(x, (fl >> 22) & 3, op.rm[2], op.rm[3], wR)));
-		else br = s_fringe_message<1, KEEP_BN>(x, kr, op.rnode, op.rm[4], wR, bnr);
+			br = matvec4_opt<false>(x.M(op.rnode), mul4(s_half<1, 0>(x, (fl >> 20) & 3, op.rm[0], op.rm[1], wR, tpos), s_half<1, 3>(x, (fl >> 22) & 3, op.rm[2], op.rm[3], wR, tpos)));
+		else br = s_fringe_message<1, KEEP_BN>(x, kr, op.rnode, op.rm[4], wR, bnr, tpos);
 		const int e_bl = EXP2 && kl == CH_CORE ? eA : 0, e_br = EXP2 && kr == CH_CORE ? eB : 0;
 		__builtin_amdgcn_s_setprio(3);
 		unsigned nw0 = 0, nw1 = 0;
 		if (i + 1 < op_end) fetch_block(i + 1, (fl >> 24) & 1);
+		if (TABLES && (fl & (1 << 8))) fetch_ctab(i + 1);
 		if (nxw > 0) nw0 = word_at(op.nx_words);
 		if (nxw > 1) nw1 = word_at(op.nx_words + ((fl >> 25) & 1 ? (int64_t)0 : (int64_t)mrow));
 		if (fl & (1 << 26)) A = lower_at(op.nx_a);
diff --git a/profiles/pre_order_cherry_count.py b/profiles/pre_order_cherry_count.py
--- /dev/null
+++ b/profiles/pre_order_cherry_count.py
@@ -0,0 +1,52 @@
+#!/usr/bin/env python3
+import collections
+import json
+import os
+import sys
+
+import numpy as np
+
+sys.path.insert(0, os.path.dirname(os.path.dirname(os.path.abspath(__file__))))
+from physher_amd import _lib, synth
+
+FP64_PER_MESSAGE = 20
+WAVES = 1e6 / 64 * 4
+
+
+def records(left, right, root):
+    lib = _lib.load()
+    left = np.ascontiguousarray(left, dtype=np.int32)
+    right = np.ascontiguousarray(right, dtype=np.int32)
+    T = (len(left) + 1) // 2
+    out = np.zeros((T, 6), dtype=np.int32)
+    n = lib.phyamd_pre_order_cherry_tables(T, left.ctypes.data, right.ctypes.data, int(root), out.ctypes.data, T)
+    if n < 0:
+        raise RuntimeError(lib.phyamd_last_error().decode())
+    return out[:n]
+
+
+def count(left, right, root):
+    recs = records(left, right, root)
+    messages, position = recs[:, 1], recs[:, 2]
+    hist = collections.Counter(messages.tolist())
+    tables = int((position > 0).sum())
+    return {"ops": int(len(recs)), "cherry_messages": int(messages.sum()), "ops_with_table": tables,
+            "messages_per_op": {str(k): hist.get(k, 0) for k in range(5)},
+            "positions": {str(k): int((position == k).sum()) for k in range(7)},
+            "still_computed": int(messages.sum()) - tables,
+            "fp64_instructions_removed_per_wave": tables * FP64_PER_MESSAGE,
+            "matrix_fetches_removed_per_wave": tables,
+            "fp64_wave_instructions_removed_per_evaluation": tables * FP64_PER_MESSAGE * WAVES}
+
+
+def main():
+    taxa = int(sys.argv[1]) if len(sys.argv) > 1 else 1000
+    seed = int(sys.argv[2]) if len(sys.argv) > 2 else 1
+    tree = synth.random_tree(taxa, np.random.default_rng(seed))
+    res = {"taxa": taxa, "seed": seed}
+    res.update(count(tree.left, tree.right, tree.root))
+    print(json.dumps(res))
+
+
+if __name__ == "__main__":
+    main()
```

After: 36.80 (median of 6 runs). No clear change (+1.0%).
